# JiangongChen/ORB_SLAM3-1

Measured on AMD Instinct MI355X. Metric: tracking frames/s (ORB extract+match), higher is better.
Workload: dtype u8; 1 GPU; ORBextractor 640x480, 8 levels, 1000 features (configs[1]) + SearchByBoW 1000x1000 per frame (configs[2]); batch_per_gpu=256

## Files before the change

### orb_slam3-1_amd/csrc/orbx_device.h

```cpp
#pragma once

#include <stddef.h>
#include <stdint.h>

#include "../../include/orbslam3_hip.h"

namespace orbx {

constexpr int kEdge = 19;
constexpr int kHalfPatch = 15;
constexpr int kPatch = 31;
constexpr int kMaxLevels = 16;
constexpr int kOctLogFactor = 6;

struct LevelDesc {
    int32_t w, h, stride;
    int32_t nfeat;
    int64_t off;
    int32_t cell_begin, cell_count;
    int32_t cand_off, cand_cap;
    int32_t sel_off, sel_cap;
    float scale;
    int32_t patch_size;
};

struct CellDesc {
    int16_t level;
    int16_t x0, y0, x1, y1;
    int32_t slot_off, slot_cap;
};

struct TileDesc {
    int16_t level, x0, y0, pad;
};

__host__ __device__ inline int xcd_grid(int n_items) { return 8 * ((n_items + 7) / 8); }
__host__ __device__ inline int xcd_remap(int block, int grid, int frame)
{
    const int chunk = grid >> 3;
    return (((block & 7) + frame) & 7) * chunk + (block >> 3);
}

__host__ __device__ inline uint32_t pack_key(uint32_t x, uint32_t y, uint32_t resp) { return (x << 20) | (y << 8) | resp; }
__host__ __device__ inline uint32_t key_x(uint32_t e) { return e >> 20; }
__host__ __device__ inline uint32_t key_y(uint32_t e) { return (e >> 8) & 0xFFFu; }
__host__ __device__ inline uint32_t key_resp(uint32_t e) { return e & 0xFFu; }

}
```

### orb_slam3-1_amd/csrc/orbx_extractor.hip

```cpp
#include <hip/hip_runtime.h>

#include <algorithm>
#include <cmath>
#include <cstdarg>
#include <cstdio>
#include <cstdlib>
#include <cstring>
#include <string>
#include <vector>

#include "hip_check.h"
#include "orbx_kernels.hip"

namespace orbx {

thread_local std::string g_last_error;

int fail(int code, const char* fmt, ...)
{
    char buf[512];
    va_list ap;
    va_start(ap, fmt);
    vsnprintf(buf, sizeof(buf), fmt, ap);
    va_end(ap);
    g_last_error = buf;
    return code;
}

static inline int cv_round_host(double v) { return (int)std::nearbyint(v); }
static inline int cv_floor_host(double v) { int i = (int)v; return i - (i > v); }
static inline int round_up(int v, int a) { return (v + a - 1) / a * a; }

static void gauss_taps_q8(int n, double sigma, int* taps)
{
    std::vector<double> k(n);
    const double scale2x = -0.5 / (sigma * sigma);
    double sum = 0;
    for (int i = 0; i < n; i++) { const double x = i - (n - 1) * 0.5; k[i] = std::exp(scale2x * x * x); sum += k[i]; }
    sum = 1. / sum;
    double err = 0;
    long long acc = 0;
    for (int i = 0; i < n / 2; i++) {
        const double adj = k[i] * sum * 256.0 + err;
        const long long v0 = cv_round_host(adj);
        err = adj - (double)v0;
        taps[i] = taps[n - 1 - i] = (int)v0;
        acc += v0;
    }
    taps[n / 2] = (int)(256 - 2 * acc);
}

template <typename T>
struct DevBuf {
    T* p = nullptr;
    size_t n = 0;
    int ensure(size_t count)
    {
        if (count <= n) return ORBX_OK;
        if (p) { (void)hipFree(p); p = nullptr; n = 0; }
        ORBX_HIP(hipMalloc((void**)&p, count * sizeof(T)));
        n = count;
        return ORBX_OK;
    }
    int upload(const std::vector<T>& v)
    {
        int r = ensure(v.size() ? v.size() : 1);
        if (r) return r;
        if (!v.empty()) ORBX_HIP(hipMemcpy(p, v.data(), v.size() * sizeof(T), hipMemcpyHostToDevice));
        return ORBX_OK;
    }
    void release() { if (p) (void)hipFree(p); p = nullptr; n = 0; }
};

}

using namespace orbx;

struct orbx_extractor {
    int device = 0;
    int nfeatures = 0, nlevels = 0, ini_th = 0, min_th = 0;
    float scale_factor_f = 0;
    double scale_factor_d = 0;
    std::vector<float> scale, inv_scale, sigma2, inv_sigma2;
    std::vector<int> nfeat;
    int taps[7];
    int max_kp = 0;

    int geo_w = 0, geo_h = 0;
    std::vector<LevelDesc> levels;
    std::vector<CellDesc> cells;
    std::vector<TileDesc> tiles;
    size_t pyr_frame_bytes = 0;
    int cand_frame_entries = 0, sel_frame_entries = 0;
    std::vector<StripDesc> strips;
    FastLds fast_layout;
    int fast_corner_cap = 0;
    size_t fast_lds = 0, oct_lds = 0;
    int oct_pool = 0, oct_lds_keys = 0, oct_small_keys = 0;
    bool oct_nodes_hbm = false;
    size_t oct_node_stride = 0;
    size_t oct_small_lds = 0;
    int oct_dyn_keys = 0;
    size_t oct_dyn_lds = 0;
    bool oct_keys_forced = false;

    DevBuf<LevelDesc> d_levels;
    DevBuf<CellDesc> d_cells;
    DevBuf<TileDesc> d_tiles;
    DevBuf<StripDesc> d_strips;
    std::vector<DevBuf<int> > d_qsx0, d_yofs;
    std::vector<DevBuf<uint4> > d_qsel, d_qalpha;
    std::vector<DevBuf<short> > d_ibeta;
    std::vector<DevBuf<int> > d_xofs;
    std::vector<DevBuf<short> > d_ialpha;
    std::vector<uint8_t> resize_generic;

    int batch_cap = 0, last_batch = 0;
    DevBuf<uint8_t> d_pyr, d_blur;
    DevBuf<uint32_t> d_cand, d_scratch, d_sel;
    DevBuf<uint8_t> d_oct_nodes;
    DevBuf<int> d_cell_count, d_sel_count, d_kp_dst;
    DevBuf<OrbxKeyPoint> d_lvl_kps;
    DevBuf<OrbxKeyPoint> d_kps;
    DevBuf<uint8_t> d_desc;
    DevBuf<int> d_n, d_mono, d_status;
    DevBuf<int> d_sad;
    DevBuf<uint8_t> d_stereo_io;
    int out_cap = 0;
    hipStream_t stream = nullptr;
    static constexpr int kProfEvents = 8;
    bool profile = false;
    hipEvent_t prof_ev[kProfEvents] = {};
    int prof_marks = 0;
    hipStream_t prof_stream = nullptr;
    hipStream_t side_stream = nullptr;
    hipEvent_t ev_fork = nullptr, ev_join = nullptr;
    hipStream_t oct_stream = nullptr;
    hipEvent_t ev_oct_join = nullptr, ev_fast0 = nullptr, ev_resize = nullptr;
    hipEvent_t ev_tail = nullptr;
    int dbg_tail_delay_us = 0;
    int last_octree_variant = 0;
    int oct_split = 0, oct_pool_hi = 0;
    size_t oct_lds_hi = 0;
    int split_parts = 1;
    bool serial_schedule = false;
    int resize_tail_first = 4;
    bool oct_dyn_off = false;
    int oct_dyn_max_batch = 64;
    int oct_dyn_keys_beside = 6144;
    bool resize_beside = true;
    std::vector<hipStream_t> aux_streams;
    hipEvent_t ev_parts_fork = nullptr;
    std::vector<hipEvent_t> ev_parts_join;

    int setup_geometry(int w, int h);
    int ensure_batch(int batch);
    int enqueue(const uint8_t* d_imgs, bool level0_ready, int batch, int row_stride, size_t frame_stride,
                int lap0, int lap1, OrbxKeyPoint* o_kps, uint8_t* o_desc, int cap, int* o_n, int* o_mono, int* o_status,
                hipStream_t st);
};

static void build_tables(orbx_extractor* e)
{
    const int nl = e->nlevels;
    e->scale.assign(nl, 1.0f); e->sigma2.assign(nl, 1.0f); e->inv_scale.resize(nl); e->inv_sigma2.resize(nl);
    for (int i = 1; i < nl; i++) {
        e->scale[i] = (float)(e->scale[i - 1] * e->scale_factor_d);
        e->sigma2[i] = e->scale[i] * e->scale[i];
    }
    for (int i = 0; i < nl; i++) {
        e->inv_scale[i] = 1.0f / e->scale[i];
        e->inv_sigma2[i] = 1.0f / e->sigma2[i];
    }
    e->nfeat.resize(nl);
    const float factor = (float)(1.0f / e->scale_factor_d);
    float per_scale = e->nfeatures * (1 - factor) / (1 - (float)std::pow((double)factor, (double)nl));
    int sum = 0;
    for (int l = 0; l < nl - 1; l++) {
        e->nfeat[l] = (int)std::nearbyintf(per_scale);
        sum += e->nfeat[l];
        per_scale *= factor;
    }
    e->nfeat[nl - 1] = std::max(e->nfeatures - sum, 0);
    e->max_kp = 0;
    for (int l = 0; l < nl; l++) e->max_kp += std::max(e->nfeat[l] + 3, 32);
    gauss_taps_q8(7, 2.0, e->taps);
}

int orbx_extractor::setup_geometry(int w, int h)
{
    if (w == geo_w && h == geo_h) return ORBX_OK;
    levels.assign(nlevels, LevelDesc());
    cells.clear();
    tiles.clear();
    strips.clear();
    size_t off = 0;
    int cand_off = 0, sel_off = 0, max_tw = 0, max_th = 0, max_nfeat = 0;
    std::vector<int> node_need(nlevels, 0);
    d_qsx0.resize(nlevels); d_yofs.resize(nlevels); d_qsel.resize(nlevels); d_qalpha.resize(nlevels); d_ibeta.resize(nlevels);
    d_xofs.resize(nlevels); d_ialpha.resize(nlevels); resize_generic.assign(nlevels, 0);
    for (int l = 0; l < nlevels; l++) {
        LevelDesc& L = levels[l];
        L.w = (int)std::nearbyintf((float)w * inv_scale[l]);
        L.h = (int)std::nearbyintf((float)h * inv_scale[l]);
        if (L.w < 1 || L.h < 1) return fail(ORBX_ERR_ARG, "pyramid level %d of a %dx%d image is empty", l, w, h);
        if (L.w > 4096 + 32 || L.h > 4096 + 32) return fail(ORBX_ERR_ARG, "image %dx%d too large (keys are 12-bit)", w, h);
        L.stride = round_up(L.w, 64);
        L.off = (int64_t)off;
        off += (size_t)L.stride * L.h;
        off = (off + 255) & ~(size_t)255;
        L.nfeat = nfeat[l];
        L.scale = scale[l];
        L.patch_size = (int)(kPatch * scale[l]);
        {
            const int bw = (L.w - kEdge + 3) - (kEdge - 3), bh = (L.h - kEdge + 3) - (kEdge - 3);
            const int n_ini = bh > 0 ? (int)std::roundf((float)bw / (float)bh) : 0;
            L.sel_off = sel_off; L.sel_cap = std::max({nfeat[l] + 3, 32, 4 * std::max(n_ini, 0)});
            node_need[l] = std::max(nfeat[l], 4 * std::max(n_ini, 0));
        }
        sel_off += (L.sel_cap + 1) & ~1;
        max_nfeat = std::max(max_nfeat, node_need[l]);
        L.cell_begin = (int)cells.size();
        L.cand_off = cand_off;
        const int minBX = kEdge - 3, minBY = minBX, maxBX = L.w - kEdge + 3, maxBY = L.h - kEdge + 3;
        const float width = (float)(maxBX - minBX), height = (float)(maxBY - minBY);
        const int nCols = (int)(width / 35.f), nRows = (int)(height / 35.f);
        if (nCols > 0 && nRows > 0) {
            const int wCell = (int)std::ceil(width / nCols), hCell = (int)std::ceil(height / nRows);
            for (int i = 0; i < nRows; i++) {
                const float iniY = (float)(minBY + i * hCell);
                float maxY = iniY + hCell + 6;
                if (iniY >= maxBY - 3) continue;
                if (maxY > maxBY) maxY = (float)maxBY;
                for (int j = 0; j < nCols; j++) {
                    const float iniX = (float)(minBX + j * wCell);
                    float maxX = iniX + wCell + 6;
                    if (iniX >= maxBX - 6) continue;
                    if (maxX > maxBX) maxX = (float)maxBX;
                    CellDesc c;
                    c.level = (int16_t)l;
                    c.x0 = (int16_t)iniX; c.x1 = (int16_t)maxX; c.y0 = (int16_t)iniY; c.y1 = (int16_t)maxY;
                    const int iw = c.x1 - c.x0 - 6, ih = c.y1 - c.y0 - 6;
                    if (iw <= 0 || ih <= 0) continue;
                    c.slot_off = cand_off;
                    c.slot_cap = ((iw + 1) / 2) * ((ih + 1) / 2);
                    cand_off += c.slot_cap;
                    max_tw = std::max(max_tw, c.x1 - c.x0);
                    max_th = std::max(max_th, c.y1 - c.y0);
                    cells.push_back(c);
                }
            }
        }
        L.cell_count = (int)cells.size() - L.cell_begin;
        L.cand_cap = cand_off - L.cand_off;
        for (int c0 = L.cell_begin; c0 < (int)cells.size();) {
            int c1 = c0 + 1;
            while (c1 < (int)cells.size() && cells[c1].y0 == cells[c0].y0) c1++;
            const int n_row = c1 - c0;
            const int w_cell = std::max(cells[c0].x1 - cells[c0].x0 - 6, 1);
            static const int strip_width = getenv("ORBX_STRIP_WIDTH") ? std::max(48, std::min(atoi(getenv("ORBX_STRIP_WIDTH")), 250)) : kStripWidth;
            const int per = std::max(1, std::min(kStripMaxCells, (strip_width - 6) / w_cell));
            const int n_strips_row = (n_row + per - 1) / per;
            for (int k = 0; k < n_strips_row; k++) {
                const int a = c0 + (int)((long long)n_row * k / n_strips_row), b = c0 + (int)((long long)n_row * (k + 1) / n_strips_row);
                StripDesc sd;
                sd.level = (int16_t)l; sd.cell0 = (int16_t)a; sd.ncell = (int16_t)(b - a);
                sd.x0 = cells[a].x0; sd.x1 = cells[b - 1].x1; sd.y0 = cells[a].y0; sd.y1 = cells[a].y1; sd.pad = 0;
                strips.push_back(sd);
            }
            c0 = c1;
        }
        for (int y0 = 0; y0 < L.h; y0 += kBlurTH)
            for (int x0 = 0; x0 < L.w; x0 += kBlurTW) {
                TileDesc t; t.level = (int16_t)l; t.x0 = (int16_t)x0; t.y0 = (int16_t)y0; t.pad = 0;
                tiles.push_back(t);
            }
        if (l > 0) {
            const LevelDesc& P = levels[l - 1];
            const double scale_x = 1. / ((double)L.w / P.w), scale_y = 1. / ((double)L.h / P.h);
            const int wpad = round_up(L.w, 4);
            std::vector<int> xofs(wpad, 0), yofs(L.h);
            std::vector<short> ia((size_t)wpad * 2, 0), ib((size_t)L.h * 2);
            auto sat = [](float v) { int iv = (int)std::nearbyintf(v); return (short)std::min(std::max(iv, -32768), 32767); };
            for (int dx = 0; dx < L.w; dx++) {
                float fx = (float)((dx + 0.5) * scale_x - 0.5);
                int sx = cv_floor_host(fx);
                fx -= sx;
                if (sx < 0) { fx = 0; sx = 0; }
                if (sx >= P.w - 1) { fx = 0; sx = P.w - 1; }
                xofs[dx] = sx;
                ia[2 * dx] = sat((1.f - fx) * 2048);
                ia[2 * dx + 1] = sat(fx * 2048);
            }
            for (int dy = 0; dy < L.h; dy++) {
                float fy = (float)((dy + 0.5) * scale_y - 0.5);
                int sy = cv_floor_host(fy);
                fy -= sy;
                yofs[dy] = sy;
                ib[2 * dy] = sat((1.f - fy) * 2048);
                ib[2 * dy + 1] = sat(fy * 2048);
            }
            const int nq = wpad / 4;
            std::vector<int> qsx0(nq);
            std::vector<uint4> qsel(nq), qal(nq);
            for (int q = 0; q < nq; q++) {
                qsx0[q] = xofs[4 * q];
                uint32_t se[4], al[4];
                for (int k = 0; k < 4; k++) {
                    const int dx = 4 * q + k;
                    if (dx < L.w) {
                        const int o = xofs[dx] - qsx0[q];
                        if (o < 0) return fail(ORBX_ERR_INTERNAL, "resize table: source offset %d", o);
                        if (o > 6) { resize_generic[l] = 1; se[k] = 0x0C0C0C0Cu; al[k] = 0u; continue; }
                        se[k] = (uint32_t)o | 0x0C000C00u | ((uint32_t)(o + 1) << 16);
                        al[k] = (uint32_t)(uint16_t)ia[2 * dx] | ((uint32_t)(uint16_t)ia[2 * dx + 1] << 16);
                    } else { se[k] = 0x0C0C0C0Cu; al[k] = 0u; }
                }
                qsel[q] = make_uint4(se[0], se[1], se[2], se[3]);
                qal[q] = make_uint4(al[0], al[1], al[2], al[3]);
            }
            int r;
            if (resize_generic[l] && ((r = d_xofs[l].upload(xofs)) || (r = d_ialpha[l].upload(ia)))) return r;
            if ((r = d_qsx0[l].upload(qsx0)) || (r = d_yofs[l].upload(yofs)) || (r = d_qsel[l].upload(qsel)) || (r = d_qalpha[l].upload(qal)) ||
                (r = d_ibeta[l].upload(ib))) return r;
        }
    }
    pyr_frame_bytes = off;
    cand_frame_entries = std::max(cand_off, 1);
    sel_frame_entries = sel_off;
    {
        if (cells.size() > 32767) return fail(ORBX_ERR_ARG, "%zu FAST cells exceed the strip table's 16-bit cell index", cells.size());
        int max_nch = 1, max_ngx = 1, max_sth = 7, max_ent = 1, max_ncell = 1, max_int = 1;
        for (const StripDesc& sd : strips) {
            const int g0 = (sd.x0 + 3) >> 2, g1 = (sd.x1 - 4) >> 2, ngx = g1 - g0 + 1, sth = sd.y1 - sd.y0, ih = sth - 6;
            if (ngx > 64 || ih > 127) return fail(ORBX_ERR_ARG, "FAST strip of %dx%d px exceeds the 64-quad x 127-row work item index", sd.x1 - sd.x0, sth);
            const int xa = (4 * (g0 - 1)) & ~15, qoff = 4 * g0 - xa;
            max_nch = std::max(max_nch, (qoff + 4 * ngx + 4 + 15) >> 4);
            for (int j = 0; j < sd.ncell; j++) { const CellDesc& c = cells[sd.cell0 + j]; max_int = std::max(max_int, (c.x1 - c.x0 - 6) * ih); }
            max_ngx = std::max(max_ngx, ngx); max_sth = std::max(max_sth, sth);
            max_ent = std::max(max_ent, ((ih + 3) / 4) * (ngx + sd.ncell - 1));
            max_ncell = std::max(max_ncell, (int)sd.ncell);
        }
        if (max_int > 8191) return fail(ORBX_ERR_ARG, "FAST cell interior of %d px exceeds the 8191-px bitmask", max_int);
        FastLds& Z = fast_layout;
        auto al16 = [](size_t v) { return (v + 15) & ~(size_t)15; };
        size_t o = 0;
        Z.tile_pitch = 16 * max_nch;
        o = al16((size_t)max_sth * Z.tile_pitch);
        Z.map_off = (int)o; Z.map_pitch = 4 * max_ngx + 8;
        o = al16(o + (size_t)(max_sth - 6 + 2) * Z.map_pitch);
        Z.colcell_off = (int)o; o = al16(o + Z.map_pitch);
        Z.ent_cap = (max_ent + 7) & ~7;
        Z.ent_off = (int)o; o = al16(o + 2 * 4 * (size_t)Z.ent_cap);
        Z.px_off = (int)o; o = al16(o + 2 * 4 * (size_t)kPxCap);
        Z.corner_cap = fast_corner_cap > 0 ? fast_corner_cap : kCornerCap;
        Z.corner_off = (int)o; o = al16(o + 2 * 4 * (size_t)Z.corner_cap);
        Z.wpc = (max_int + 31) / 32;
        Z.pre_off = (int)o; o = al16(o + 4 * (size_t)max_ncell * Z.wpc);
        Z.bits_off = (int)o; o = al16(o + 4 * (size_t)max_ncell * Z.wpc);
        Z.total = (int)o;
        fast_lds = o;
        if (fast_lds > 150 * 1024) return fail(ORBX_ERR_ARG, "FAST strip of %d quads x %d rows does not fit LDS", max_ngx, max_sth);
    }
    oct_pool = max_nfeat + 16;
    if (oct_pool > 32000) return fail(ORBX_ERR_ARG, "nfeatures per level %d too large for the device octree (16-bit node ids)", max_nfeat);
    const char* env = getenv("ORBX_OCT_LDS_KEYS");
    oct_lds_keys = env ? atoi(env) : 0;
    oct_keys_forced = env != nullptr;
    auto pool_bytes = [](int pool) { return (size_t)pool * (2 * sizeof(SortNode) + 8 + 16 + 2 * kOctLogFactor) + (size_t)((pool + 15) & ~15); };
    const size_t node_bytes = pool_bytes(oct_pool);
    oct_split = 0; oct_pool_hi = 0; oct_lds_hi = 0;
    {
        size_t best = (size_t)nlevels * node_bytes;
        for (int sp = 1; sp < nlevels; sp++) {
            int hi = 0;
            for (int l = sp; l < nlevels; l++) hi = std::max(hi, node_need[l]);
            const size_t cost = (size_t)sp * node_bytes + (size_t)(nlevels - sp) * pool_bytes(hi + 16);
            if (cost < best) { best = cost; oct_split = sp; oct_pool_hi = hi + 16; oct_lds_hi = pool_bytes(hi + 16) + 16; }
        }
    }
    oct_nodes_hbm = node_bytes > 150 * 1024;
    oct_node_stride = (node_bytes + 255) & ~(size_t)255;
    if (oct_nodes_hbm) oct_lds_keys = 0;
    if (!oct_nodes_hbm && node_bytes + 8 * (size_t)oct_lds_keys > 150 * 1024) oct_lds_keys = (int)((150 * 1024 - node_bytes) / 8);
    if (oct_lds_keys < 0) oct_lds_keys = 0;
    oct_lds = node_bytes + 8 * (size_t)oct_lds_keys + 16;
    int max_cand_cap = 0;
    for (const LevelDesc& lv : levels) max_cand_cap = std::max(max_cand_cap, lv.cand_cap);
    oct_small_keys = max_cand_cap;
    if (oct_nodes_hbm || node_bytes + 8 * (size_t)oct_small_keys > 150 * 1024) oct_small_keys = 0;
    oct_small_lds = node_bytes + 8 * (size_t)oct_small_keys + 16;
    if (oct_lds_keys > 0 && oct_lds_keys < max_cand_cap) oct_lds_keys = 0;
    oct_dyn_keys = 0; oct_dyn_lds = 0;
    if (!oct_nodes_hbm && oct_small_keys == 0 && node_bytes + 8 * 2048 <= 150 * 1024) {
        oct_dyn_keys = (int)std::min<size_t>((size_t)max_cand_cap, (150 * 1024 - node_bytes) / 8);
        if (const char* envd = getenv("ORBX_OCT_DYN_KEYS")) oct_dyn_keys = std::max(64, std::min(oct_dyn_keys, atoi(envd)));
        oct_dyn_lds = node_bytes + 8 * (size_t)oct_dyn_keys + 16;
    }
    if (!oct_nodes_hbm) {
        ORBX_HIP(hipFuncSetAttribute((const void*)k_octree<false>, hipFuncAttributeMaxDynamicSharedMemorySize, (int)node_bytes + 64));
        ORBX_HIP(hipFuncSetAttribute((const void*)k_octree<true>, hipFuncAttributeMaxDynamicSharedMemorySize, (int)std::max(oct_lds, oct_small_lds)));
        if (oct_dyn_keys > 0) ORBX_HIP(hipFuncSetAttribute((const void*)k_octree_dyn, hipFuncAttributeMaxDynamicSharedMemorySize, (int)oct_dyn_lds));
    } else {
        oct_lds = 64; oct_small_lds = 64;
    }
    ORBX_HIP(hipFuncSetAttribute((const void*)k_fast_strips, hipFuncAttributeMaxDynamicSharedMemorySize, (int)fast_lds));
    int r;
    if ((r = d_levels.upload(levels)) || (r = d_cells.upload(cells)) || (r = d_tiles.upload(tiles)) || (r = d_strips.upload(strips))) return r;
    geo_w = w; geo_h = h;
    batch_cap = 0;
    return ORBX_OK;
}

int orbx_extractor::ensure_batch(int batch)
{
    if (batch <= batch_cap) return ORBX_OK;
    int r;
    const size_t B = (size_t)batch;
    if ((r = d_pyr.ensure(B * pyr_frame_bytes + 64)) || (r = d_blur.ensure(B * pyr_frame_bytes + 64)) ||
        (r = d_cand.ensure(B * cand_frame_entries)) || (r = d_scratch.ensure(B * 2 * cand_frame_entries)) ||
        (r = d_sel.ensure(B * sel_frame_entries)) || (r = d_cell_count.ensure(B * std::max<size_t>(cells.size(), 1))) ||
        (r = d_sel_count.ensure(B * nlevels)) || (r = d_kp_dst.ensure(B * sel_frame_entries)) ||
        (r = d_lvl_kps.ensure(B * sel_frame_entries)) || (r = d_n.ensure(B)) || (r = d_mono.ensure(B)) || (r = d_status.ensure(B)))
        return r;
    if (oct_nodes_hbm && (r = d_oct_nodes.ensure(B * nlevels * oct_node_stride))) return r;
    ORBX_HIP(hipMemset(d_pyr.p, 0, B * pyr_frame_bytes + 64));
    ORBX_HIP(hipMemset(d_blur.p, 0, B * pyr_frame_bytes + 64));
    batch_cap = batch;
    return ORBX_OK;
}

namespace orbx {
__global__ void k_debug_spin(long long ticks)
{
    const long long t0 = wall_clock64();
    while (wall_clock64() - t0 < ticks) __builtin_amdgcn_s_sleep(32);
}
__global__ __launch_bounds__(256) void k_copy_level0(const uint8_t* __restrict__ src, int row_stride, size_t src_frame_stride,
                                                     uint8_t* __restrict__ pyr, size_t frame_stride, LevelDesc L)
{
    const int x4 = (blockIdx.x * blockDim.x + threadIdx.x) * 4;
    const int y = blockIdx.y;
    if (x4 >= L.w) return;
    const uint8_t* s = src + (size_t)blockIdx.z * src_frame_stride + (size_t)y * row_stride + x4;
    uint32_t v = 0;
#pragma unroll
    for (int k = 0; k < 4; k++) if (x4 + k < L.w) v |= (uint32_t)s[k] << (8 * k);
    *(uint32_t*)(pyr + (size_t)blockIdx.z * frame_stride + L.off + (size_t)y * L.stride + x4) = v;
}
}

int orbx_extractor::enqueue(const uint8_t* d_imgs, bool level0_ready, int batch, int row_stride, size_t frame_stride,
                            int lap0, int lap1, OrbxKeyPoint* o_kps, uint8_t* o_desc, int cap, int* o_n, int* o_mono, int* o_status,
                            hipStream_t st)
{
    const int B = batch;
    ORBX_HIP(hipMemsetAsync(o_status, 0, sizeof(int) * B, st));
    int mark_i = 0;
    auto mark = [&]() { if (profile && mark_i < kProfEvents) (void)hipEventRecord(prof_ev[mark_i++], st); };
#define ORBX_LAUNCHED(name) do { const hipError_t le_ = hipGetLastError(); if (le_ != hipSuccess) return fail(ORBX_ERR_HIP, "launch of %s: %s", name, hipGetErrorString(le_)); } while (0)
    const bool in_place = !level0_ready && ((uintptr_t)d_imgs % 16 == 0) && (row_stride % 16 == 0) && (frame_stride % 16 == 0);
    const int n_cells = (int)cells.size();
    const int quads = (sel_frame_entries + 7) / 8;

    auto run_range = [&](int f0, int nB, hipStream_t s, hipStream_t blur_s, bool marks) -> int {
        uint8_t* pyr = d_pyr.p + (size_t)f0 * pyr_frame_bytes;
        uint8_t* blr = d_blur.p + (size_t)f0 * pyr_frame_bytes;
        SrcImage lvl0;
        lvl0.base = nullptr; lvl0.frame_stride = 0; lvl0.stride = 0; lvl0.w = levels[0].w; lvl0.h = levels[0].h;
        if (in_place) { lvl0.base = d_imgs + (size_t)f0 * frame_stride; lvl0.frame_stride = frame_stride; lvl0.stride = row_stride; }
        if (marks) mark();
        if (!level0_ready && !in_place) {
            const LevelDesc& L0 = levels[0];
            dim3 g((L0.w / 4 + 255) / 256, L0.h, nB);
            hipLaunchKernelGGL(k_copy_level0, g, dim3(256), 0, s, d_imgs + (size_t)f0 * frame_stride, row_stride, frame_stride, pyr, pyr_frame_bytes, L0);
            ORBX_LAUNCHED("k_copy_level0");
        }
        if (marks) mark();
        int l_tail = (nB >= 64 && resize_tail_first >= 2 && resize_tail_first < nlevels) ? resize_tail_first : nlevels;
        for (int l = l_tail; l < nlevels; l++) if (resize_generic[l]) l_tail = nlevels;
        const bool chain_beside = resize_beside && blur_s && oct_stream && n_cells > 0 && l_tail < nlevels && l_tail > 1 &&
                                  !strips.empty() && strips[0].level == 0;
        hipStream_t rs = chain_beside ? oct_stream : s;
        if (chain_beside) { ORBX_HIP(hipEventRecord(ev_fork, s)); ORBX_HIP(hipStreamWaitEvent(rs, ev_fork, 0)); }
        for (int l = 1; l < l_tail; l++) {
            const LevelDesc& D = levels[l];
            dim3 g(xcd_grid(((D.w + kResizeTW - 1) / kResizeTW) * ((D.h + kResizeRows - 1) / kResizeRows)), nB);
            const LevelDesc& P = levels[l - 1];
            SrcImage src;
            src.base = pyr + P.off; src.frame_stride = pyr_frame_bytes; src.stride = P.stride; src.w = P.w; src.h = P.h;
            if (l == 1 && in_place) src = lvl0;
            if (resize_generic[l])
                hipLaunchKernelGGL(k_resize_generic, dim3((D.w + 255) / 256, D.h, nB), dim3(256), 0, rs, src, pyr, pyr_frame_bytes, D,
                                   d_xofs[l].p, d_ialpha[l].p, d_yofs[l].p, d_ibeta[l].p);
            else
            hipLaunchKernelGGL(k_resize, g, dim3(256), 0, rs, src, pyr, pyr_frame_bytes, D,
                               d_qsx0[l].p, d_qsel[l].p, d_qalpha[l].p, d_yofs[l].p, d_ibeta[l].p);
            ORBX_LAUNCHED("k_resize");
        }
        if (chain_beside) ORBX_HIP(hipEventRecord(ev_resize, rs));
        const bool small_batch = !oct_keys_forced && oct_small_keys > 0 && (long long)B * nlevels <= 512;
        const bool dyn_keys = !oct_keys_forced && !small_batch && oct_dyn_keys > 0 && B <= oct_dyn_max_batch && !oct_dyn_off;
        const int dyn_k = (blur_s && B >= 32) ? std::min(oct_dyn_keys, oct_dyn_keys_beside) : oct_dyn_keys;
        const size_t o_lds = small_batch ? oct_small_lds : (dyn_keys ? oct_dyn_lds - 8 * (size_t)(oct_dyn_keys - dyn_k) : oct_lds);
        const int o_keys = small_batch ? oct_small_keys : (dyn_keys ? dyn_k : oct_lds_keys);
        uint32_t* sel = d_sel.p + (size_t)f0 * sel_frame_entries;
        int* sel_cnt = d_sel_count.p + (size_t)f0 * nlevels;
        int* kp_dst = d_kp_dst.p + (size_t)f0 * sel_frame_entries;
        auto oct_kernel = oct_nodes_hbm ? k_octree<false, false> : (dyn_keys ? k_octree_dyn : (o_keys > 0 ? k_octree<true, true> : k_octree<false, true>));
        const bool two_launches = !oct_nodes_hbm && (o_keys == 0 || dyn_keys) && oct_split > 0 && oct_stream && blur_s;
        const int lv_lo = two_launches ? oct_split : nlevels;
        auto launch_octree = [&](hipStream_t qs, int lv0, int lv1, size_t lds, int pool, int keys) {
            if (lv1 > lv0)
                hipLaunchKernelGGL(oct_kernel, dim3(lv1 - lv0, nB), dim3(64), lds, qs, d_levels.p, d_cells.p, d_cand.p + (size_t)f0 * cand_frame_entries, (size_t)cand_frame_entries,
                                   d_cell_count.p + (size_t)f0 * std::max<size_t>(cells.size(), 1), n_cells, d_scratch.p + (size_t)f0 * 2 * cand_frame_entries, (size_t)2 * cand_frame_entries, pool, keys,
                                   sel, sel_frame_entries, sel_cnt, nlevels, o_status + f0,
                                   d_oct_nodes.p ? d_oct_nodes.p + (size_t)f0 * nlevels * oct_node_stride : nullptr, oct_node_stride, lv0);
        };
        auto launch_blur = [&](hipStream_t bs) {
            hipLaunchKernelGGL(k_blur, dim3(xcd_grid((int)tiles.size()), nB), dim3(256), 0, bs, lvl0, pyr, in_place ? pyr : nullptr, blr, pyr_frame_bytes,
                               d_levels.p, d_tiles.p, (int)tiles.size(), taps[0], taps[1], taps[2], taps[3]);
        };
        bool oct0_early = false;
        bool tail_beside = false;
        uint32_t* cand = d_cand.p + (size_t)f0 * cand_frame_entries;
        int* cell_cnt = d_cell_count.p + (size_t)f0 * std::max<size_t>(cells.size(), 1);
        auto launch_fast = [&](hipStream_t fs, int s0, int s1) {
            if (s1 > s0)
                hipLaunchKernelGGL(k_fast_strips, dim3(xcd_grid(s1 - s0), nB), dim3(256), fast_lds, fs, lvl0, pyr, pyr_frame_bytes, d_levels.p, d_cells.p,
                                   d_strips.p + s0, s1 - s0, n_cells, ini_th, min_th, fast_layout, cand, (size_t)cand_frame_entries, cell_cnt);
        };
        int tail_strip = (int)strips.size();
        for (int si = (int)strips.size() - 1; si >= 0 && strips[si].level >= l_tail; si--) tail_strip = si;
        if (l_tail < nlevels) {
            ResizeTables T;
            std::memset(&T, 0, sizeof(T));
            for (int l = l_tail; l < nlevels; l++) { T.q_sx0[l] = d_qsx0[l].p; T.q_sel[l] = d_qsel[l].p; T.q_alpha[l] = d_qalpha[l].p; T.yofs[l] = d_yofs[l].p; T.ibeta[l] = d_ibeta[l].p; }
            const bool beside = blur_s && oct_stream && n_cells > 0 && tail_strip > 0;
            hipStream_t ts = beside ? oct_stream : s;
            if (beside && !chain_beside) { ORBX_HIP(hipEventRecord(ev_fork, s)); ORBX_HIP(hipStreamWaitEvent(ts, ev_fork, 0)); }
            if (dbg_tail_delay_us > 0) hipLaunchKernelGGL(k_debug_spin, dim3(1), dim3(64), 0, ts, (long long)dbg_tail_delay_us * 100);
            hipLaunchKernelGGL(k_resize_tail, dim3(nB), dim3(1024), 0, ts, pyr, pyr_frame_bytes, d_levels.p, T, l_tail, nlevels);
            ORBX_LAUNCHED("k_resize_tail");
            if (beside) {
                ORBX_HIP(hipEventRecord(ev_tail, ts));
                tail_beside = true;
                launch_fast(ts, tail_strip, (int)strips.size());
                ORBX_HIP(hipEventRecord(ev_oct_join, ts));
                int l1_strip = tail_strip;
                for (int si = tail_strip - 1; si >= 0 && strips[si].level >= 1; si--) l1_strip = si;
                if (two_launches && oct_split > 1 && l1_strip > 0 && l1_strip < tail_strip) {
                    launch_fast(s, 0, l1_strip);
                    ORBX_HIP(hipEventRecord(ev_fast0, s));
                    ORBX_HIP(hipStreamWaitEvent(blur_s, ev_fast0, 0));
                    launch_octree(blur_s, 0, 1, o_lds, oct_pool, o_keys);
                    oct0_early = true;
                    if (chain_beside) ORBX_HIP(hipStreamWaitEvent(s, ev_resize, 0));
                    launch_fast(s, l1_strip, tail_strip);
                } else if (chain_beside && l1_strip > 0 && l1_strip < tail_strip) {
                    launch_fast(s, 0, l1_strip);
                    ORBX_HIP(hipStreamWaitEvent(s, ev_resize, 0));
                    launch_fast(s, l1_strip, tail_strip);
                } else {
                    if (chain_beside) ORBX_HIP(hipStreamWaitEvent(s, ev_resize, 0));
                    launch_fast(s, 0, tail_strip);
                }
                ORBX_HIP(hipStreamWaitEvent(blur_s, ev_oct_join, 0));
            } else {
                if (marks) mark();
                if (n_cells > 0) launch_fast(s, 0, (int)strips.size());
            }
        } else {
            if (marks) mark();
            if (n_cells > 0) launch_fast(s, 0, (int)strips.size());
        }
        ORBX_LAUNCHED("k_fast_strips");
        if (marks) mark();
        hipStream_t os = blur_s ? blur_s : s;
        if (blur_s) {
            ORBX_HIP(hipEventRecord(ev_fork, s));
            ORBX_HIP(hipStreamWaitEvent(blur_s, ev_fork, 0));
        }
        if (two_launches) {
            ORBX_HIP(hipStreamWaitEvent(oct_stream, ev_fork, 0));
            {
                const int k_hi = dyn_keys ? std::max(64, o_keys / 2) : 0;
                launch_octree(oct_stream, oct_split, nlevels, oct_lds_hi + 8 * (size_t)k_hi, oct_pool_hi, k_hi);
            }
            ORBX_HIP(hipEventRecord(ev_oct_join, oct_stream));
        }
        launch_octree(os, oct0_early ? 1 : 0, lv_lo, o_lds, oct_pool, o_keys);
        if (blur_s) {
            if (tail_beside) ORBX_HIP(hipStreamWaitEvent(s, ev_tail, 0));
            launch_blur(s);
        }
        last_octree_variant = (oct_nodes_hbm ? 0 : (dyn_keys ? 3 : (o_keys > 0 ? 1 : 2))) | (two_launches ? 4 : 0) | (oct0_early ? 8 : 0) | (in_place ? 16 : 0) | (tail_beside ? 32 : 0) | (chain_beside ? 64 : 0);
        if (two_launches) ORBX_HIP(hipStreamWaitEvent(os, ev_oct_join, 0));
        ORBX_LAUNCHED("k_octree / k_blur");
        if (marks) mark();
        hipLaunchKernelGGL(k_index, dim3(nB), dim3(64), 0, os, d_levels.p, nlevels, sel, sel_frame_entries, sel_cnt,
                           lap0, lap1, cap, kp_dst, sel_frame_entries, o_n + f0, o_mono + f0, o_status + f0);
        ORBX_LAUNCHED("k_index");
        if (marks) mark();
        if (blur_s) { ORBX_HIP(hipEventRecord(ev_join, blur_s)); ORBX_HIP(hipStreamWaitEvent(s, ev_join, 0)); }
        else launch_blur(s);
        if (marks) mark();
        hipLaunchKernelGGL(k_orient_desc, dim3((unsigned)(((long long)quads * nB + 7) / 8 * 8)), dim3(256), 0, s, pyr, blr, pyr_frame_bytes,
                           d_levels.p, nlevels, sel, sel_frame_entries, sel_cnt, kp_dst, sel_frame_entries,
                           o_kps + (size_t)f0 * cap, o_desc + (size_t)f0 * cap * 32, cap, d_lvl_kps.p + (size_t)f0 * sel_frame_entries, quads, nB);
        ORBX_LAUNCHED("k_orient_desc");
        if (marks) mark();
        return ORBX_OK;
    };

    int parts = 1;
    if (!profile && split_parts > 1 && B >= 32 * split_parts) parts = std::min(split_parts, 1 + (int)aux_streams.size());
    int r;
    if (parts == 1) {
        if ((r = run_range(0, B, st, (!profile && !serial_schedule && side_stream && B >= 32) ? side_stream : nullptr, true))) return r;
    } else {
        ORBX_HIP(hipEventRecord(ev_parts_fork, st));
        for (int p = 0; p < parts; p++) {
            const int f0 = (int)((long long)B * p / parts), f1 = (int)((long long)B * (p + 1) / parts);
            hipStream_t s = p == 0 ? st : aux_streams[p - 1];
            if (p > 0) ORBX_HIP(hipStreamWaitEvent(s, ev_parts_fork, 0));
            if ((r = run_range(f0, f1 - f0, s, nullptr, false))) return r;
            if (p > 0) { ORBX_HIP(hipEventRecord(ev_parts_join[p - 1], s)); ORBX_HIP(hipStreamWaitEvent(st, ev_parts_join[p - 1], 0)); }
        }
    }
    prof_marks = mark_i;
    prof_stream = st;
    ORBX_HIP(hipGetLastError());
    last_batch = B;
    return ORBX_OK;
}

extern "C" {

int orbx_profile_enable(orbx_extractor* e, int on)
{
    if (!e) return fail(ORBX_ERR_ARG, "NULL handle");
    ORBX_HIP(hipSetDevice(e->device));
    if (on && !e->prof_ev[0])
        for (int i = 0; i < orbx_extractor::kProfEvents; i++) ORBX_HIP(hipEventCreate(&e->prof_ev[i]));
    e->profile = on != 0;
    e->prof_marks = 0;
    return ORBX_OK;
}

int orbx_profile_read(orbx_extractor* e, float* stage_ms, int n_stages)
{
    if (!e || !stage_ms) return fail(ORBX_ERR_ARG, "NULL argument");
    if (!e->profile || e->prof_marks < 2) return fail(ORBX_ERR_ARG, "profiling was not enabled for the last call");
    ORBX_HIP(hipSetDevice(e->device));
    ORBX_HIP(hipStreamSynchronize(e->prof_stream));
    for (int i = 0; i < n_stages; i++) {
        stage_ms[i] = 0.f;
        if (i + 1 < e->prof_marks) ORBX_HIP(hipEventElapsedTime(&stage_ms[i], e->prof_ev[i], e->prof_ev[i + 1]));
    }
    return ORBX_OK;
}

const char* orbx_last_error(void) { return g_last_error.c_str(); }

int orbx_device_count(void)
{
    int n = 0;
    if (hipGetDeviceCount(&n) != hipSuccess) return 0;
    return n;
}

int orbx_create(int nfeatures, float scale_factor, int nlevels, int ini_th_fast, int min_th_fast, int device, orbx_extractor** out)
{
    if (!out) return fail(ORBX_ERR_ARG, "out is NULL");
    *out = nullptr;
    if (nlevels < 1 || nlevels > kMaxLevels || nfeatures < 1 || !(scale_factor > 1.0f))
        return fail(ORBX_ERR_ARG, "bad extractor parameters (nfeatures=%d scale=%f nlevels=%d)", nfeatures, scale_factor, nlevels);
    if (int r = stage::check_device(device)) return r;
    ORBX_HIP(hipSetDevice(device));
    orbx_extractor* e = new orbx_extractor();
    e->device = device;
    e->nfeatures = nfeatures; e->nlevels = nlevels; e->ini_th = ini_th_fast; e->min_th = min_th_fast;
    e->scale_factor_f = scale_factor; e->scale_factor_d = (double)scale_factor;
    build_tables(e);
    if (hipStreamCreateWithFlags(&e->stream, hipStreamNonBlocking) != hipSuccess) { delete e; return fail(ORBX_ERR_HIP, "stream create failed"); }
    if (hipStreamCreateWithFlags(&e->side_stream, hipStreamNonBlocking) != hipSuccess ||
        hipEventCreateWithFlags(&e->ev_fork, hipEventDisableTiming) != hipSuccess ||
        hipEventCreateWithFlags(&e->ev_join, hipEventDisableTiming) != hipSuccess ||
        hipEventCreateWithFlags(&e->ev_parts_fork, hipEventDisableTiming) != hipSuccess ||
        hipStreamCreateWithFlags(&e->oct_stream, hipStreamNonBlocking) != hipSuccess ||
        hipEventCreateWithFlags(&e->ev_oct_join, hipEventDisableTiming) != hipSuccess ||
        hipEventCreateWithFlags(&e->ev_tail, hipEventDisableTiming) != hipSuccess ||
        hipEventCreateWithFlags(&e->ev_resize, hipEventDisableTiming) != hipSuccess ||
        hipEventCreateWithFlags(&e->ev_fast0, hipEventDisableTiming) != hipSuccess) { orbx_destroy(e); return fail(ORBX_ERR_HIP, "side stream create failed"); }
    if (const char* env = getenv("ORBX_SERIAL")) e->serial_schedule = atoi(env) != 0;
    if (const char* env = getenv("ORBX_SPLIT")) e->split_parts = std::max(1, std::min(atoi(env), 4));
    if (const char* env = getenv("ORBX_RESIZE_TAIL")) e->resize_tail_first = atoi(env);
    if (const char* env = getenv("ORBX_RESIZE_BESIDE")) e->resize_beside = atoi(env) != 0;
    if (const char* env = getenv("ORBX_OCT_DYN")) e->oct_dyn_off = atoi(env) == 0;
    if (const char* env = getenv("ORBX_OCT_DYN_MAXB")) e->oct_dyn_max_batch = atoi(env);
    if (const char* env = getenv("ORBX_OCT_DYN_KEYS_BESIDE")) e->oct_dyn_keys_beside = std::max(64, atoi(env));
    for (int i = 0; i + 1 < e->split_parts; i++) {
        hipStream_t s = nullptr; hipEvent_t ev = nullptr;
        if (hipStreamCreateWithFlags(&s, hipStreamNonBlocking) != hipSuccess || hipEventCreateWithFlags(&ev, hipEventDisableTiming) != hipSuccess) {
            if (s) (void)hipStreamDestroy(s);
            break;
        }
        e->aux_streams.push_back(s); e->ev_parts_join.push_back(ev);
    }
    *out = e;
    return ORBX_OK;
}

void orbx_destroy(orbx_extractor* e)
{
    if (!e) return;
    (void)hipSetDevice(e->device);
    if (e->stream) { (void)hipStreamSynchronize(e->stream); (void)hipStreamDestroy(e->stream); }
    if (e->side_stream) { (void)hipStreamSynchronize(e->side_stream); (void)hipStreamDestroy(e->side_stream); }
    if (e->oct_stream) { (void)hipStreamSynchronize(e->oct_stream); (void)hipStreamDestroy(e->oct_stream); }
    if (e->ev_oct_join) (void)hipEventDestroy(e->ev_oct_join);
    if (e->ev_fast0) (void)hipEventDestroy(e->ev_fast0);
    if (e->ev_resize) (void)hipEventDestroy(e->ev_resize);
    if (e->ev_tail) (void)hipEventDestroy(e->ev_tail);
    if (e->ev_fork) (void)hipEventDestroy(e->ev_fork);
    if (e->ev_join) (void)hipEventDestroy(e->ev_join);
    for (hipStream_t s : e->aux_streams) { (void)hipStreamSynchronize(s); (void)hipStreamDestroy(s); }
    for (hipEvent_t ev : e->ev_parts_join) (void)hipEventDestroy(ev);
    if (e->ev_parts_fork) (void)hipEventDestroy(e->ev_parts_fork);
    e->d_levels.release(); e->d_cells.release(); e->d_tiles.release(); e->d_strips.release();
    for (auto& b : e->d_qsx0) b.release();
    for (auto& b : e->d_yofs) b.release();
    for (auto& b : e->d_qsel) b.release();
    for (auto& b : e->d_qalpha) b.release();
    for (auto& b : e->d_ibeta) b.release();
    for (auto& b : e->d_xofs) b.release();
    for (auto& b : e->d_ialpha) b.release();
    e->d_pyr.release(); e->d_blur.release(); e->d_cand.release(); e->d_scratch.release(); e->d_sel.release(); e->d_oct_nodes.release();
    e->d_cell_count.release(); e->d_sel_count.release(); e->d_kp_dst.release(); e->d_lvl_kps.release();
    e->d_kps.release(); e->d_desc.release(); e->d_n.release(); e->d_mono.release(); e->d_status.release();
    e->d_sad.release(); e->d_stereo_io.release();
    delete e;
}

int orbx_max_keypoints(const orbx_extractor* e) { return e ? e->max_kp : 0; }

int orbx_max_keypoints_for(const orbx_extractor* e, int width, int height)
{
    if (!e || width < 1 || height < 1) return 0;
    int total = 0;
    for (int l = 0; l < e->nlevels; l++) {
        const int lw = (int)std::nearbyintf((float)width * e->inv_scale[l]), lh = (int)std::nearbyintf((float)height * e->inv_scale[l]);
        const int bw = (lw - kEdge + 3) - (kEdge - 3), bh = (lh - kEdge + 3) - (kEdge - 3);
        const int n_ini = bh > 0 ? (int)std::roundf((float)bw / (float)bh) : 0;
        total += std::max({e->nfeat[l] + 3, 32, 4 * std::max(n_ini, 0)});
    }
    return total;
}
int orbx_levels(const orbx_extractor* e) { return e ? e->nlevels : 0; }
float orbx_scale_factor(const orbx_extractor* e) { return e ? e->scale_factor_f : 0.f; }

int orbx_scale_tables(const orbx_extractor* e, float* scale, float* inv_scale, float* sigma2, float* inv_sigma2)
{
    if (!e) return fail(ORBX_ERR_ARG, "NULL handle");
    for (int i = 0; i < e->nlevels; i++) {
        if (scale) scale[i] = e->scale[i];
        if (inv_scale) inv_scale[i] = e->inv_scale[i];
        if (sigma2) sigma2[i] = e->sigma2[i];
        if (inv_sigma2) inv_sigma2[i] = e->inv_sigma2[i];
    }
    return ORBX_OK;
}

int orbx_features_per_level(const orbx_extractor* e, int* n_per_level)
{
    if (!e || !n_per_level) return fail(ORBX_ERR_ARG, "NULL argument");
    for (int i = 0; i < e->nlevels; i++) n_per_level[i] = e->nfeat[i];
    return ORBX_OK;
}

int orbx_extract_batch_device(orbx_extractor* e, const uint8_t* d_imgs, int batch, int width, int height,
                              int row_stride, size_t frame_stride, int lap0, int lap1,
                              OrbxKeyPoint* d_kps, uint8_t* d_desc, int cap, int32_t* d_n, int32_t* d_mono,
                              int32_t* d_status, void* stream)
{
    if (!e || !d_imgs || !d_kps || !d_desc || !d_n || !d_mono || !d_status) return fail(ORBX_ERR_ARG, "NULL argument");
    if (batch < 1 || width < 1 || height < 1 || row_stride < width || cap < 1) return fail(ORBX_ERR_ARG, "bad batch/geometry");
    ORBX_HIP(hipSetDevice(e->device));
    int r;
    if ((r = e->setup_geometry(width, height)) || (r = e->ensure_batch(batch))) return r;
    return e->enqueue(d_imgs, false, batch, row_stride, frame_stride, lap0, lap1, d_kps, d_desc, cap, d_n, d_mono, d_status,
                      (hipStream_t)stream);
}

int orbx_extract_batch(orbx_extractor* e, const uint8_t* const* imgs, int batch, int width, int height, int stride,
                       int lap0, int lap1, OrbxKeyPoint* kps, uint8_t* desc, int cap, int* n, int* mono_index)
{
    if (!e || !imgs || !kps || !desc || !n || !mono_index) return fail(ORBX_ERR_ARG, "NULL argument");
    if (batch < 1 || cap < 1) return fail(ORBX_ERR_ARG, "bad batch/capacity");
    if (width < 1 || height < 1) { for (int b = 0; b < batch; b++) { n[b] = 0; mono_index[b] = -1; } return ORBX_ERR_EMPTY; }
    if (stride < width) return fail(ORBX_ERR_ARG, "stride < width");
    ORBX_HIP(hipSetDevice(e->device));
    int r;
    if ((r = e->setup_geometry(width, height)) || (r = e->ensure_batch(batch))) return r;
    const size_t B = (size_t)batch;
    if ((r = e->d_kps.ensure(B * cap)) || (r = e->d_desc.ensure(B * cap * 32))) return r;
    const LevelDesc& L0 = e->levels[0];
    for (int b = 0; b < batch; b++) {
        if (!imgs[b]) return fail(ORBX_ERR_ARG, "imgs[%d] is NULL", b);
        ORBX_HIP(hipMemcpy2DAsync(e->d_pyr.p + b * e->pyr_frame_bytes + L0.off, L0.stride, imgs[b], stride, width, height,
                                  hipMemcpyHostToDevice, e->stream));
    }
    if ((r = e->enqueue(nullptr, true, batch, 0, 0, lap0, lap1, e->d_kps.p, e->d_desc.p, cap, e->d_n.p, e->d_mono.p, e->d_status.p, e->stream)))
        return r;
    std::vector<int> st(batch);
    ORBX_HIP(hipMemcpyAsync(n, e->d_n.p, sizeof(int) * B, hipMemcpyDeviceToHost, e->stream));
    ORBX_HIP(hipMemcpyAsync(mono_index, e->d_mono.p, sizeof(int) * B, hipMemcpyDeviceToHost, e->stream));
    ORBX_HIP(hipMemcpyAsync(st.data(), e->d_status.p, sizeof(int) * B, hipMemcpyDeviceToHost, e->stream));
    ORBX_HIP(hipMemcpyAsync(kps, e->d_kps.p, sizeof(OrbxKeyPoint) * B * cap, hipMemcpyDeviceToHost, e->stream));
    ORBX_HIP(hipMemcpyAsync(desc, e->d_desc.p, B * cap * 32, hipMemcpyDeviceToHost, e->stream));
    ORBX_HIP(hipStreamSynchronize(e->stream));
    for (int b = 0; b < batch; b++)
        if (st[b] != ORBX_OK) return fail(st[b], "frame %d: device status %d (n=%d, cap=%d)", b, st[b], n[b], cap);
    return ORBX_OK;
}

int orbx_extract(orbx_extractor* e, const uint8_t* img, int width, int height, int stride,
                 int lap0, int lap1, OrbxKeyPoint* kps, uint8_t* desc, int cap, int* n, int* mono_index)
{
    if (!img || width < 1 || height < 1) {
        if (n) *n = 0;
        if (mono_index) *mono_index = -1;
        return ORBX_ERR_EMPTY;
    }
    const uint8_t* imgs[1] = {img};
    return orbx_extract_batch(e, imgs, 1, width, height, stride, lap0, lap1, kps, desc, cap, n, mono_index);
}

int orbx_pyramid_level_size(const orbx_extractor* e, int level, int* width, int* height)
{
    if (!e || level < 0 || level >= e->nlevels || e->geo_w == 0) return fail(ORBX_ERR_ARG, "no pyramid (level %d)", level);
    if (width) *width = e->levels[level].w;
    if (height) *height = e->levels[level].h;
    return ORBX_OK;
}

static int download_level(orbx_extractor* e, const uint8_t* base, int frame, int level, int border, uint8_t* dst, int dst_stride)
{
    if (!e || !dst || level < 0 || level >= e->nlevels || frame < 0 || frame >= e->last_batch || border < 0)
        return fail(ORBX_ERR_ARG, "bad frame/level");
    const LevelDesc& L = e->levels[level];
    if (dst_stride < L.w + 2 * border) return fail(ORBX_ERR_ARG, "dst_stride too small");
    ORBX_HIP(hipSetDevice(e->device));
    ORBX_HIP(hipStreamSynchronize(e->stream));
    ORBX_HIP(hipMemcpy2D(dst + (size_t)border * dst_stride + border, dst_stride, base + (size_t)frame * e->pyr_frame_bytes + L.off,
                         L.stride, L.w, L.h, hipMemcpyDeviceToHost));
    if (border > 0) {
        auto refl = [](int p, int len) { if (len == 1) return 0; while (p < 0 || p >= len) p = p < 0 ? -p : 2 * len - 2 - p; return p; };
        for (int y = 0; y < L.h + 2 * border; y++) {
            const int sy = refl(y - border, L.h) + border;
            uint8_t* row = dst + (size_t)y * dst_stride;
            const uint8_t* srow = dst + (size_t)sy * dst_stride;
            if (sy != y) std::memcpy(row + border, srow + border, L.w);
            for (int x = 0; x < border; x++) {
                row[x] = row[border + refl(x - border, L.w)];
                row[border + L.w + x] = row[border + refl(L.w + x, L.w)];
            }
        }
    }
    return ORBX_OK;
}

int orbx_pyramid_level(orbx_extractor* e, int frame, int level, int border, uint8_t* dst, int dst_stride)
{
    return download_level(e, e ? e->d_pyr.p : nullptr, frame, level, border, dst, dst_stride);
}

int orbx_debug_blurred_level(orbx_extractor* e, int frame, int level, uint8_t* dst, int dst_stride)
{
    return download_level(e, e ? e->d_blur.p : nullptr, frame, level, 0, dst, dst_stride);
}

int orbx_debug_candidates(orbx_extractor* e, int frame, int level, OrbxKeyPoint* out, int cap, int* n)
{
    if (!e || !out || !n || level < 0 || level >= e->nlevels || frame < 0 || frame >= e->last_batch) return fail(ORBX_ERR_ARG, "bad frame/level");
    ORBX_HIP(hipSetDevice(e->device));
    ORBX_HIP(hipStreamSynchronize(e->stream));
    const LevelDesc& L = e->levels[level];
    std::vector<int> cnt(std::max(L.cell_count, 1));
    std::vector<uint32_t> ent(std::max(L.cand_cap, 1));
    if (L.cell_count > 0) {
        ORBX_HIP(hipMemcpy(cnt.data(), e->d_cell_count.p + (size_t)frame * e->cells.size() + L.cell_begin, sizeof(int) * L.cell_count, hipMemcpyDeviceToHost));
        ORBX_HIP(hipMemcpy(ent.data(), e->d_cand.p + (size_t)frame * e->cand_frame_entries + L.cand_off, sizeof(uint32_t) * L.cand_cap, hipMemcpyDeviceToHost));
    }
    int k = 0;
    for (int c = 0; c < L.cell_count; c++) {
        const CellDesc& cd = e->cells[L.cell_begin + c];
        for (int i = 0; i < cnt[c]; i++, k++) {
            if (k >= cap) continue;
            const uint32_t en = ent[cd.slot_off - L.cand_off + i];
            OrbxKeyPoint kp;
            kp.x = (float)key_x(en); kp.y = (float)key_y(en); kp.size = 7.f; kp.angle = -1.f; kp.response = (float)key_resp(en);
            kp.octave = 0; kp.class_id = -1;
            out[k] = kp;
        }
    }
    *n = k;
    return ORBX_OK;
}

int orbx_debug_level_keypoints(orbx_extractor* e, int frame, int level, OrbxKeyPoint* out, int cap, int* n)
{
    if (!e || !out || !n || level < 0 || level >= e->nlevels || frame < 0 || frame >= e->last_batch) return fail(ORBX_ERR_ARG, "bad frame/level");
    ORBX_HIP(hipSetDevice(e->device));
    ORBX_HIP(hipStreamSynchronize(e->stream));
    const LevelDesc& L = e->levels[level];
    int cnt = 0;
    ORBX_HIP(hipMemcpy(&cnt, e->d_sel_count.p + (size_t)frame * e->nlevels + level, sizeof(int), hipMemcpyDeviceToHost));
    *n = cnt;
    const int m = std::min(cnt, cap);
    if (m > 0)
        ORBX_HIP(hipMemcpy(out, e->d_lvl_kps.p + (size_t)frame * e->sel_frame_entries + L.sel_off, sizeof(OrbxKeyPoint) * m, hipMemcpyDeviceToHost));
    return ORBX_OK;
}

int orbx_debug_set_tail_delay(orbx_extractor* e, int microseconds)
{
    if (!e || microseconds < 0 || microseconds > 20000) return fail(ORBX_ERR_ARG, "bad tail delay");
    e->dbg_tail_delay_us = microseconds;
    return ORBX_OK;
}

int orbx_debug_last_schedule(orbx_extractor* e)
{
    if (!e) return fail(ORBX_ERR_ARG, "NULL handle");
    return e->last_octree_variant;
}

int orbx_debug_set_fast_corner_cap(orbx_extractor* e, int cap)
{
    if (!e) return fail(ORBX_ERR_ARG, "NULL handle");
    e->fast_corner_cap = cap > 0 ? std::min(cap, 4096) : 0;
    e->geo_w = e->geo_h = 0;
    return ORBX_OK;
}

int orbx_debug_introsort(int32_t* count, int32_t* ulx, int32_t* node, int n)
{
    if (n < 0) return ORBX_ERR_ARG;
    std::vector<SortNode> v(n);
    for (int i = 0; i < n; i++) { v[i].count = count[i]; v[i].ulx = ulx[i]; v[i].node = node[i]; }
    std::vector<int> stack(3 * kIntrosortStack);
    introsort_nodes(v.data(), n, stack.data());
    for (int i = 0; i < n; i++) { count[i] = v[i].count; ulx[i] = v[i].ulx; node[i] = v[i].node; }
    return ORBX_OK;
}

int orbx_debug_wave_sort(int32_t* count, int32_t* ulx, int32_t* node, int n)
{
    if (n < 0 || n > 4000) return fail(ORBX_ERR_ARG, "n %d outside 0..4000", n);
    if (n == 0) return ORBX_OK;
    std::vector<SortNode> v(n);
    for (int i = 0; i < n; i++) { v[i].count = count[i]; v[i].ulx = ulx[i]; v[i].node = node[i]; }
    SortNode* d = nullptr;
    ORBX_HIP(hipMalloc(&d, sizeof(SortNode) * n));
    int r = ORBX_OK;
    const size_t lds = 2 * sizeof(SortNode) * (size_t)n + 2 * (size_t)n + 16;
    if (hipMemcpy(d, v.data(), sizeof(SortNode) * n, hipMemcpyHostToDevice) != hipSuccess) r = ORBX_ERR_HIP;
    if (!r && hipFuncSetAttribute((const void*)k_debug_wave_sort, hipFuncAttributeMaxDynamicSharedMemorySize, (int)lds) != hipSuccess) r = ORBX_ERR_HIP;
    if (!r) {
        hipLaunchKernelGGL(k_debug_wave_sort, dim3(1), dim3(64), lds, 0, d, n);
        if (hipGetLastError() != hipSuccess || hipDeviceSynchronize() != hipSuccess) r = ORBX_ERR_HIP;
    }
    if (!r && hipMemcpy(v.data(), d, sizeof(SortNode) * n, hipMemcpyDeviceToHost) != hipSuccess) r = ORBX_ERR_HIP;
    (void)hipFree(d);
    if (r) return fail(r, "device sort failed");
    for (int i = 0; i < n; i++) { count[i] = v[i].count; ulx[i] = v[i].ulx; node[i] = v[i].node; }
    return ORBX_OK;
}

static int stereo_enqueue(orbx_extractor* l, orbx_extractor* r, int frame0, int batch,
                          const OrbxKeyPoint* d_kps_l, const uint8_t* d_desc_l, const int32_t* d_n_l,
                          const OrbxKeyPoint* d_kps_r, const uint8_t* d_desc_r, const int32_t* d_n_r, int cap,
                          float mb, float mbf, float* d_u_right, float* d_depth, hipStream_t st)
{
    if (l->geo_w == 0 || l->geo_w != r->geo_w || l->geo_h != r->geo_h || l->nlevels != r->nlevels || l->scale_factor_f != r->scale_factor_f)
        return fail(ORBX_ERR_ARG, "the two extractors do not hold pyramids of the same geometry");
    if (l->device != r->device) return fail(ORBX_ERR_ARG, "the two extractors live on different devices");
    if (frame0 < 0 || batch < 1 || frame0 + batch > l->last_batch || frame0 + batch > r->last_batch) return fail(ORBX_ERR_ARG, "frames outside the last extract call");
    if (l->nlevels > 16) return fail(ORBX_ERR_ARG, "more than 16 pyramid levels");
    if (cap < 1 || cap > 8192) return fail(ORBX_ERR_ARG, "cap %d outside 1..8192", cap);
    if (!(mb > 0.f) || !(mbf > 0.f)) return fail(ORBX_ERR_ARG, "mb and mbf must be positive");
    int rr = l->d_sad.ensure((size_t)batch * cap);
    if (rr) return rr;
    StereoTables T;
    for (int i = 0; i < 16; i++) { T.scale[i] = l->scale[std::min(i, l->nlevels - 1)]; T.inv_scale[i] = l->inv_scale[std::min(i, l->nlevels - 1)]; }
    const uint8_t* pl = l->d_pyr.p + (size_t)frame0 * l->pyr_frame_bytes;
    const uint8_t* pr = r->d_pyr.p + (size_t)frame0 * r->pyr_frame_bytes;
    hipLaunchKernelGGL(k_stereo_match, dim3((cap + 3) / 4, batch), dim3(256), 0, st, pl, pr, l->pyr_frame_bytes, l->d_levels.p, T,
                       d_kps_l, d_desc_l, d_n_l, d_kps_r, d_desc_r, d_n_r, cap, mb, mbf, l->nlevels, d_u_right, d_depth, l->d_sad.p);
    int n_pow2 = 2;
    while (n_pow2 < cap) n_pow2 <<= 1;
    hipLaunchKernelGGL(k_stereo_median, dim3(batch), dim3(256), (size_t)n_pow2 * sizeof(int), st, d_n_l, cap, n_pow2, d_u_right, d_depth, l->d_sad.p);
    ORBX_HIP(hipGetLastError());
    return ORBX_OK;
}

int orbx_stereo_matches_device(orbx_extractor* left, orbx_extractor* right, int batch,
                               const OrbxKeyPoint* d_kps_l, const uint8_t* d_desc_l, const int32_t* d_n_l,
                               const OrbxKeyPoint* d_kps_r, const uint8_t* d_desc_r, const int32_t* d_n_r, int cap,
                               float mb, float mbf, float* d_u_right, float* d_depth, void* stream)
{
    if (!left || !right || !d_kps_l || !d_desc_l || !d_n_l || !d_kps_r || !d_desc_r || !d_n_r || !d_u_right || !d_depth) return fail(ORBX_ERR_ARG, "NULL argument");
    ORBX_HIP(hipSetDevice(left->device));
    return stereo_enqueue(left, right, 0, batch, d_kps_l, d_desc_l, d_n_l, d_kps_r, d_desc_r, d_n_r, cap, mb, mbf, d_u_right, d_depth, (hipStream_t)stream);
}

int orbx_stereo_matches(orbx_extractor* left, orbx_extractor* right, int frame,
                        const OrbxKeyPoint* kps_l, const uint8_t* desc_l, int n_l,
                        const OrbxKeyPoint* kps_r, const uint8_t* desc_r, int n_r, float mb, float mbf, float* u_right, float* depth)
{
    if (!left || !right || n_l < 0 || n_r < 0 || (n_l > 0 && (!kps_l || !desc_l || !u_right || !depth)) || (n_r > 0 && (!kps_r || !desc_r)))
        return fail(ORBX_ERR_ARG, "NULL argument");
    if (n_l == 0) return ORBX_OK;
    ORBX_HIP(hipSetDevice(left->device));
    const int cap = std::max(std::max(n_l, n_r), 1);
    auto al = [](size_t v) { return (v + 255) & ~(size_t)255; };
    const size_t o_kl = 0, o_dl = al(o_kl + sizeof(OrbxKeyPoint) * (size_t)cap), o_kr = al(o_dl + 32 * (size_t)cap), o_dr = al(o_kr + sizeof(OrbxKeyPoint) * (size_t)cap),
                 o_n = al(o_dr + 32 * (size_t)cap), o_u = al(o_n + 8), o_d = al(o_u + 4 * (size_t)cap), total = al(o_d + 4 * (size_t)cap);
    int r = left->d_stereo_io.ensure(total);
    if (r) return r;
    uint8_t* b = left->d_stereo_io.p;
    hipStream_t st = left->stream;
    const int32_t nn[2] = {n_l, n_r};
    ORBX_HIP(hipMemcpyAsync(b + o_kl, kps_l, sizeof(OrbxKeyPoint) * (size_t)n_l, hipMemcpyHostToDevice, st));
    ORBX_HIP(hipMemcpyAsync(b + o_dl, desc_l, 32 * (size_t)n_l, hipMemcpyHostToDevice, st));
    if (n_r > 0) {
        ORBX_HIP(hipMemcpyAsync(b + o_kr, kps_r, sizeof(OrbxKeyPoint) * (size_t)n_r, hipMemcpyHostToDevice, st));
        ORBX_HIP(hipMemcpyAsync(b + o_dr, desc_r, 32 * (size_t)n_r, hipMemcpyHostToDevice, st));
    }
    ORBX_HIP(hipMemcpyAsync(b + o_n, nn, 8, hipMemcpyHostToDevice, st));
    ORBX_HIP(hipStreamSynchronize(right->stream));
    r = stereo_enqueue(left, right, frame, 1, (const OrbxKeyPoint*)(b + o_kl), b + o_dl, (const int32_t*)(b + o_n),
                       (const OrbxKeyPoint*)(b + o_kr), b + o_dr, (const int32_t*)(b + o_n) + 1, cap, mb, mbf, (float*)(b + o_u), (float*)(b + o_d), st);
    if (r) return r;
    ORBX_HIP(hipMemcpyAsync(u_right, b + o_u, 4 * (size_t)n_l, hipMemcpyDeviceToHost, st));
    ORBX_HIP(hipMemcpyAsync(depth, b + o_d, 4 * (size_t)n_l, hipMemcpyDeviceToHost, st));
    ORBX_HIP(hipStreamSynchronize(st));
    return ORBX_OK;
}

float orbx_debug_fast_atan2(float y, float x) { return fast_atan2_deg(y, x); }
void orbx_debug_sincos(float a, float* c, float* s) { sincos_f32(a, c, s); }

#ifdef ORBX_FAST_TIMING
int orbx_debug_fast_prof(unsigned long long* out16)
{
    unsigned long long z[16] = {0};
    if (hipMemcpyFromSymbol(out16, HIP_SYMBOL(d_fast_prof), sizeof(z)) != hipSuccess) return ORBX_ERR_HIP;
    if (hipMemcpyToSymbol(HIP_SYMBOL(d_fast_prof), z, sizeof(z)) != hipSuccess) return ORBX_ERR_HIP;
    return ORBX_OK;
}
#endif
#ifdef ORBX_OCT_TIMING
int orbx_debug_oct_prof(unsigned long long* out10)
{
    if (hipMemcpyFromSymbol(out10, HIP_SYMBOL(d_oct_prof), 10 * sizeof(unsigned long long)) != hipSuccess) return ORBX_ERR_HIP;
    return ORBX_OK;
}
#endif


}
```

### orb_slam3-1_amd/csrc/orbx_kernels.hip

```cpp
#include <hip/hip_runtime.h>
#include <stdint.h>

#include "orbx_device.h"
#include "orbx_introsort.h"
#include "orbx_math.h"

namespace orbx {

__device__ __align__(16) const signed char d_pattern[1024] = {
#include "orb_pattern_31.inc"
};

typedef unsigned short us2 __attribute__((ext_vector_type(2)));
__device__ __forceinline__ us2 as_us2(uint32_t v) { return __builtin_bit_cast(us2, v); }
__device__ __forceinline__ uint32_t as_u32(us2 v) { return __builtin_bit_cast(uint32_t, v); }

struct SrcImage {
    const uint8_t* base;
    size_t frame_stride;
    int32_t stride, w, h;
};

struct __attribute__((aligned(4))) Dwords3 { uint32_t x, y, z; };
struct __attribute__((aligned(4))) Dwords4 { uint32_t x, y, z, w; };
constexpr int kResizeRows = 64, kResizeTW = 64;

__device__ __forceinline__ void resize_tile(const SrcImage& src, uint8_t* __restrict__ pyr, size_t frame_stride, const LevelDesc& dst,
                                            const int* __restrict__ q_sx0, const uint4* __restrict__ q_sel, const uint4* __restrict__ q_alpha,
                                            const int* __restrict__ yofs, const short* __restrict__ ibeta, int tile, int frame, int lane, int wave)
{
    const int tiles_x = (dst.w + kResizeTW - 1) / kResizeTW;
    const int ty = tile / tiles_x, tx = tile - ty * tiles_x;
    const int q = tx * (kResizeTW / 4) + (lane & 15), rsel = lane >> 4;
    if (4 * q >= dst.w) return;
    const int sx0 = q_sx0[q];
    const uint4 sel = q_sel[q], al = q_alpha[q];
    const uint32_t sels[4] = {sel.x, sel.y, sel.z, sel.w}, als[4] = {al.x, al.y, al.z, al.w};
    const int a = sx0 & ~3;
    const uint32_t sh = (uint32_t)(sx0 & 3);
    const int last = src.stride - 4;
    const int o0 = a, o1 = min(a + 4, last), o2 = min(a + 8, last);
    const uint8_t* S = src.base + (size_t)frame * src.frame_stride;
    uint8_t* D = pyr + (size_t)frame * frame_stride + dst.off + 4 * q;
    constexpr int NR = kResizeRows / 16;
    const int dy0 = ty * kResizeRows + wave * (kResizeRows / 4) + rsel;
    uint32_t u[NR][3], v[NR][3], bb[NR];
#pragma unroll
    for (int r = 0; r < NR; r++) {
        const int dy = min(dy0 + 4 * r, dst.h - 1);
        const int sy = yofs[dy];
        const int sy0 = min(max(sy, 0), src.h - 1), sy1 = min(max(sy + 1, 0), src.h - 1);
        bb[r] = ((const uint32_t*)ibeta)[dy];
        const uint8_t* r0p = S + (size_t)sy0 * src.stride;
        const uint8_t* r1p = S + (size_t)sy1 * src.stride;
        if (a + 8 <= last) {
            const Dwords3 tu = *(const Dwords3*)(r0p + a), tv = *(const Dwords3*)(r1p + a);
            u[r][0] = tu.x; u[r][1] = tu.y; u[r][2] = tu.z;
            v[r][0] = tv.x; v[r][1] = tv.y; v[r][2] = tv.z;
        } else {
            u[r][0] = *(const uint32_t*)(r0p + o0); u[r][1] = *(const uint32_t*)(r0p + o1); u[r][2] = *(const uint32_t*)(r0p + o2);
            v[r][0] = *(const uint32_t*)(r1p + o0); v[r][1] = *(const uint32_t*)(r1p + o1); v[r][2] = *(const uint32_t*)(r1p + o2);
        }
    }
#pragma unroll
    for (int r = 0; r < NR; r++) {
        const int dy = dy0 + 4 * r;
        if (dy >= dst.h) continue;
        const uint32_t b0 = bb[r] & 0xFFFFu, b1 = bb[r] >> 16;
        const uint32_t ulo = __builtin_amdgcn_alignbyte(u[r][1], u[r][0], sh), uhi = __builtin_amdgcn_alignbyte(u[r][2], u[r][1], sh);
        const uint32_t vlo = __builtin_amdgcn_alignbyte(v[r][1], v[r][0], sh), vhi = __builtin_amdgcn_alignbyte(v[r][2], v[r][1], sh);
        uint32_t out[4];
#pragma unroll
        for (int k = 0; k < 4; k++) {
            const us2 ak = as_us2(als[k]);
            const uint32_t h0 = __builtin_amdgcn_udot2(as_us2(__builtin_amdgcn_perm(uhi, ulo, sels[k])), ak, 0u, false);
            const uint32_t h1 = __builtin_amdgcn_udot2(as_us2(__builtin_amdgcn_perm(vhi, vlo, sels[k])), ak, 0u, false);
            const uint32_t val = ((__umul24(b0, h0 >> 4) >> 16) + (__umul24(b1, h1 >> 4) >> 16) + 2u) >> 2;
            out[k] = min(val, 255u);
        }
        *(uint32_t*)(D + (size_t)dy * dst.stride) = out[0] | (out[1] << 8) | (out[2] << 16) | (out[3] << 24);
    }
}

__global__ __launch_bounds__(256) void k_resize(SrcImage src, uint8_t* __restrict__ pyr, size_t frame_stride, LevelDesc dst,
                                                const int* __restrict__ q_sx0, const uint4* __restrict__ q_sel, const uint4* __restrict__ q_alpha,
                                                const int* __restrict__ yofs, const short* __restrict__ ibeta)
{
    const int tiles_x = (dst.w + kResizeTW - 1) / kResizeTW, tiles_y = (dst.h + kResizeRows - 1) / kResizeRows;
    const int tile = xcd_remap(blockIdx.x, gridDim.x, blockIdx.y);
    if (tile >= tiles_x * tiles_y) return;
    resize_tile(src, pyr, frame_stride, dst, q_sx0, q_sel, q_alpha, yofs, ibeta, tile, blockIdx.y, threadIdx.x & 63,
                __builtin_amdgcn_readfirstlane(threadIdx.x >> 6));
}

__global__ __launch_bounds__(256) void k_resize_generic(SrcImage src, uint8_t* __restrict__ pyr, size_t frame_stride, LevelDesc dst,
                                                        const int* __restrict__ xofs, const short* __restrict__ ialpha,
                                                        const int* __restrict__ yofs, const short* __restrict__ ibeta)
{
    const int dx = blockIdx.x * blockDim.x + threadIdx.x, dy = blockIdx.y, frame = blockIdx.z;
    if (dx >= dst.w) return;
    const uint8_t* S = src.base + (size_t)frame * src.frame_stride;
    const int sx = xofs[dx], sy = yofs[dy];
    const uint32_t a0 = (uint16_t)ialpha[2 * dx], a1 = (uint16_t)ialpha[2 * dx + 1];
    const uint32_t b0 = (uint16_t)ibeta[2 * dy], b1 = (uint16_t)ibeta[2 * dy + 1];
    const int sy0 = min(max(sy, 0), src.h - 1), sy1 = min(max(sy + 1, 0), src.h - 1);
    const int sx1 = min(sx + 1, src.w - 1);
    const uint8_t* r0 = S + (size_t)sy0 * src.stride;
    const uint8_t* r1 = S + (size_t)sy1 * src.stride;
    const uint32_t h0 = r0[sx] * a0 + r0[sx1] * a1, h1 = r1[sx] * a0 + r1[sx1] * a1;
    const uint32_t val = ((__umul24(b0, h0 >> 4) >> 16) + (__umul24(b1, h1 >> 4) >> 16) + 2u) >> 2;
    pyr[(size_t)frame * frame_stride + dst.off + (size_t)dy * dst.stride + dx] = (uint8_t)min(val, 255u);
}

struct ResizeTables {
    const int* q_sx0[kMaxLevels]; const uint4* q_sel[kMaxLevels]; const uint4* q_alpha[kMaxLevels];
    const int* yofs[kMaxLevels]; const short* ibeta[kMaxLevels];
};
__global__ __launch_bounds__(1024) void k_resize_tail(uint8_t* __restrict__ pyr, size_t frame_stride, const LevelDesc* __restrict__ levels,
                                                      ResizeTables T, int l_first, int n_levels)
{
    const int frame = blockIdx.x;
    const int sub = __builtin_amdgcn_readfirstlane(threadIdx.x >> 8), wave = __builtin_amdgcn_readfirstlane((threadIdx.x >> 6) & 3);
    const int lane = threadIdx.x & 63;
    for (int l = l_first; l < n_levels; l++) {
        const LevelDesc D = levels[l], P = levels[l - 1];
        SrcImage src;
        src.base = pyr + P.off; src.frame_stride = frame_stride; src.stride = P.stride; src.w = P.w; src.h = P.h;
        const int tiles = ((D.w + kResizeTW - 1) / kResizeTW) * ((D.h + kResizeRows - 1) / kResizeRows);
        for (int t = sub; t < tiles; t += 4)
            resize_tile(src, pyr, frame_stride, D, T.q_sx0[l], T.q_sel[l], T.q_alpha[l], T.yofs[l], T.ibeta[l], t, frame, lane, wave);
        __syncthreads();
    }
}

#include "orbx_fast_strips.inc"

#ifdef ORBX_OCT_TIMING
__device__ unsigned long long d_oct_prof[10];
#endif
struct OctLds {
    short* ulx; short* uly; short* brx; short* bry;
    int* beg; int* cnt;
    int* pidx; short* freelist; short* order;
    short* plog;
    uint8_t* flg;
};

template <bool LDS_KEYS, bool LDS_NODES>
__device__ __forceinline__ void octree_body(const LevelDesc* __restrict__ levels, const CellDesc* __restrict__ cells,
                                            const uint32_t* __restrict__ cand, size_t cand_frame_stride,
                                            const int* __restrict__ cell_count, int n_cells,
                                            uint32_t* __restrict__ scratch, size_t scratch_frame_stride,
                                            int pool, int lds_keys_cap,
                                            uint32_t* __restrict__ sel, int sel_frame_stride,
                                            int* __restrict__ sel_count, int n_levels, int* __restrict__ status,
                                            uint8_t* __restrict__ node_scratch, size_t node_stride, int level_first,
                                            uint8_t* __restrict__ smem, int* __restrict__ s_sort_stack)
{
    static_assert(LDS_NODES || !LDS_KEYS, "a pool too large for LDS leaves no room for LDS keys");
    const int level = level_first + blockIdx.x, frame = blockIdx.y;
    const int lane = threadIdx.x;
    const LevelDesc L = levels[level];
    const int N = L.nfeat;
    const unsigned long long lt = (1ull << lane) - 1ull;
#ifdef ORBX_OCT_TIMING
    long long tq[8] = {0, 0, 0, 0, 0, 0, 0, 0};
    const bool timed = level == 0 && frame == 0 && lane == 0;
    long long t_prev = clock64();
    const long long t_kernel0 = t_prev;
    int n_div = 0;
#define ORBX_OTICK(k) if (timed) { const long long t_now = clock64(); tq[k] += t_now - t_prev; t_prev = t_now; }
#else
#define ORBX_OTICK(k)
#endif

    OctLds S;
    uint8_t* p;
    if constexpr (LDS_NODES) p = smem;
    else p = node_scratch + ((size_t)blockIdx.y * gridDim.x + blockIdx.x) * node_stride;
    SortNode* const ex_new = (SortNode*)p; p += sizeof(SortNode) * pool;
    SortNode* const ex_sorted = (SortNode*)p; p += sizeof(SortNode) * pool;
    S.beg = (int*)p; p += 4 * pool;
    S.cnt = (int*)p; p += 4 * pool;
    S.ulx = (short*)p; p += 2 * pool;  S.uly = (short*)p; p += 2 * pool;
    S.brx = (short*)p; p += 2 * pool;  S.bry = (short*)p; p += 2 * pool;
    S.pidx = (int*)p; p += 4 * pool;
    S.freelist = (short*)p; p += 2 * pool; S.order = (short*)p; p += 2 * pool;
    S.plog = (short*)p; p += 2 * kOctLogFactor * pool;
    S.flg = p; p += (pool + 15) & ~15;
    uint32_t* kb;
    int cap;
    if constexpr (LDS_KEYS) { kb = (uint32_t*)p; cap = lds_keys_cap; }
    else { kb = scratch + (size_t)frame * scratch_frame_stride + 2 * (size_t)L.cand_off; cap = L.cand_cap; }

    int* out_count = sel_count + (size_t)frame * n_levels + level;
    uint32_t* out = sel + (size_t)frame * sel_frame_stride + L.sel_off;

    const uint32_t* fc = cand + (size_t)frame * cand_frame_stride;
    const int* cc = cell_count + (size_t)frame * n_cells;
    int total = 0;
    for (int c0 = 0; c0 < L.cell_count; c0 += 64) {
        const int ci = c0 + lane;
        int n = 0, slot_off = 0;
        if (ci < L.cell_count) { n = cc[L.cell_begin + ci]; slot_off = cells[L.cell_begin + ci].slot_off; }
        const int incl = wave_incl_scan(n);
        const int base = total + incl - n;
        if (base + n > cap) n = 0;
        for (int k = 0; __ballot(k < n) != 0ull; k += 8) {
            uint32_t e[8];
#pragma unroll
            for (int u = 0; u < 8; u++) e[u] = (k + u < n) ? fc[slot_off + k + u] : 0u;
#pragma unroll
            for (int u = 0; u < 8; u++) if (k + u < n) kb[base + k + u] = e[u];
        }
        total += __builtin_amdgcn_readlane(incl, 63);
    }
    if (total > cap) {
        if (lane == 0) { atomicExch(status + frame, ORBX_ERR_INTERNAL); *out_count = 0; }
        return;
    }
    __syncthreads();
    ORBX_OTICK(0)

    const int width = (L.w - kEdge + 3) - (kEdge - 3), height = (L.h - kEdge + 3) - (kEdge - 3);
    const int nIni = (height > 0) ? (int)roundf((float)width / (float)height) : 0;
    if (total == 0 || nIni <= 0 || nIni > pool / 2) {
        if (lane == 0) {
            *out_count = 0;
            if (total != 0 && nIni > pool / 2) atomicExch(status + frame, ORBX_ERR_INTERNAL);
        }
        return;
    }

    const int plog_cap = kOctLogFactor * pool;
    int np = 0, size = 0, nfree = pool, n_ex = 0;
    for (int i = lane; i < pool; i += 64) S.freelist[i] = (short)(pool - 1 - i);
    __syncthreads();
    bool overflow = false;
    auto compact = [&]() {
        int w = 0;
        for (int i0 = 0; i0 < np; i0 += 64) {
            const int i = i0 + lane;
            const int id = (i < np) ? (int)S.plog[i] : -1;
            const unsigned long long m = __ballot(id >= 0);
            if (id >= 0) { const int pos = w + __popcll(m & lt); S.plog[pos] = (short)id; S.pidx[id] = pos; }
            w += __popcll(m);
        }
        np = w;
        __syncthreads();
    };

    const float hX = (float)width / (float)nIni;
    if (nIni == 1) {
        if (lane == 0) {
            const int id = S.freelist[nfree - 1];
            S.ulx[id] = 0; S.uly[id] = 0; S.brx[id] = (short)(int)hX; S.bry[id] = (short)height;
            S.beg[id] = 0; S.cnt[id] = total; S.flg[id] = (uint8_t)(total == 1 ? 1 : 0);
            S.plog[0] = (short)id; S.pidx[id] = 0;
        }
        nfree--; np = 1; size = 1;
        __syncthreads();
    } else {
        int strip_beg = 0;
        for (int s = 0; s < nIni; s++) {
            int cnt = 0;
            for (int k0 = 0; k0 < total; k0 += 64) {
                const int k = k0 + lane;
                bool in = false;
                uint32_t e = 0;
                if (k < total) { e = kb[k]; in = ((int)((float)key_x(e) / hX) == s); }
                const unsigned long long m = __ballot(in);
                if (in) kb[cap + strip_beg + cnt + __popcll(m & lt)] = e;
                cnt += __popcll(m);
            }
            int id = -1;
            if (cnt > 0) {
                id = S.freelist[--nfree];
                if (lane == 0) {
                    S.ulx[id] = (short)(int)(hX * (float)s);       S.uly[id] = 0;
                    S.brx[id] = (short)(int)(hX * (float)(s + 1)); S.bry[id] = (short)height;
                    S.beg[id] = strip_beg; S.cnt[id] = cnt;
                    S.flg[id] = (uint8_t)(2 | (cnt == 1 ? 1 : 0));
                }
            }
            if (lane == 0) S.order[s] = (short)id;
            strip_beg += cnt;
        }
        __syncthreads();
        for (int s = nIni - 1; s >= 0; s--) {
            const int id = S.order[s];
            if (id >= 0) { if (lane == 0) { S.plog[np] = (short)id; S.pidx[id] = np; } np++; size++; }
        }
        __syncthreads();
    }
    ORBX_OTICK(1)

    auto divide_batch = [&](const int id, const bool sorted_phase, int& n_to_expand) -> bool {
        const bool act = id >= 0;
        int ulx = 0, uly = 0, brx = 0, bry = 0, beg = 0, cnt = 0, src = 0;
        if (act) {
            ulx = S.ulx[id]; uly = S.uly[id]; brx = S.brx[id]; bry = S.bry[id];
            beg = S.beg[id]; cnt = S.cnt[id]; src = (S.flg[id] >> 1) & 1;
        }
        const int halfX = (brx - ulx + 1) >> 1;
        const int halfY = (bry - uly + 1) >> 1;
        const int midx = ulx + halfX, midy = uly + halfY;
        const int in_off = (src ? cap : 0) + beg, out_off = (src ? 0 : cap) + beg;
        const unsigned long long m_act = __ballot(act);
        const int small_max = (__popcll(m_act) <= 6) ? 0 : 32;
        const bool small = act && cnt <= small_max;
        int c0 = 0, c1 = 0, c2 = 0, c3 = 0;
        if (__ballot(small) != 0ull) {
            for (int k = 0; __ballot(small && k < cnt) != 0ull; k += 4) {
#pragma unroll
                for (int u = 0; u < 4; u++) {
                    if (small && k + u < cnt) {
                        const uint32_t e = kb[in_off + k + u];
                        const int cls = ((int)key_x(e) >= midx ? 1 : 0) + ((int)key_y(e) >= midy ? 2 : 0);
                        c0 += cls == 0; c1 += cls == 1; c2 += cls == 2; c3 += cls == 3;
                    }
                }
            }
            int w0 = out_off, w1 = out_off + c0, w2 = w1 + c1, w3 = w2 + c2;
            for (int k = 0; __ballot(small && k < cnt) != 0ull; k += 4) {
                uint32_t e[4];
#pragma unroll
                for (int u = 0; u < 4; u++) e[u] = (small && k + u < cnt) ? kb[in_off + k + u] : 0u;
#pragma unroll
                for (int u = 0; u < 4; u++) {
                    if (small && k + u < cnt) {
                        const bool r = (int)key_x(e[u]) >= midx, d = (int)key_y(e[u]) >= midy;
                        const int pos = d ? (r ? w3 : w2) : (r ? w1 : w0);
                        kb[pos] = e[u];
                        w0 += (!d && !r); w1 += (!d && r); w2 += (d && !r); w3 += (d && r);
                    }
                }
            }
        }
        for (unsigned long long mb = __ballot(act && !small); mb != 0ull; mb &= mb - 1ull) {
            const int b = __builtin_ctzll(mb);
            const int bin = __builtin_amdgcn_readlane(in_off, b), bout = __builtin_amdgcn_readlane(out_off, b);
            const int bcnt = __builtin_amdgcn_readlane(cnt, b);
            const int bmx = __builtin_amdgcn_readlane(midx, b), bmy = __builtin_amdgcn_readlane(midy, b);
            int s0 = 0, s1 = 0, s2 = 0, s3 = 0;
            if (bcnt <= 64) {
                int cls = -1;
                uint32_t e = 0;
                if (lane < bcnt) { e = kb[bin + lane]; cls = ((int)key_x(e) >= bmx ? 1 : 0) + ((int)key_y(e) >= bmy ? 2 : 0); }
                const unsigned long long m0 = __ballot(cls == 0), m1 = __ballot(cls == 1), m2 = __ballot(cls == 2), m3 = __ballot(cls == 3);
                s0 = __popcll(m0); s1 = __popcll(m1); s2 = __popcll(m2); s3 = __popcll(m3);
                const unsigned long long mm = (cls == 0) ? m0 : (cls == 1) ? m1 : (cls == 2) ? m2 : m3;
                const int basec = (cls == 0) ? 0 : (cls == 1) ? s0 : (cls == 2) ? s0 + s1 : s0 + s1 + s2;
                if (cls >= 0) kb[bout + basec + __popcll(mm & lt)] = e;
            } else {
                for (int k0 = 0; k0 < bcnt; k0 += 256) {
                    uint32_t e[4];
#pragma unroll
                    for (int u = 0; u < 4; u++) { const int k = k0 + 64 * u + lane; e[u] = (k < bcnt) ? kb[bin + k] : 0u; }
#pragma unroll
                    for (int u = 0; u < 4; u++) {
                        const int k = k0 + 64 * u + lane;
                        const int cls = (k < bcnt) ? ((int)key_x(e[u]) >= bmx ? 1 : 0) + ((int)key_y(e[u]) >= bmy ? 2 : 0) : -1;
                        s0 += __popcll(__ballot(cls == 0)); s1 += __popcll(__ballot(cls == 1));
                        s2 += __popcll(__ballot(cls == 2)); s3 += __popcll(__ballot(cls == 3));
                    }
                }
                int w0 = bout, w1 = bout + s0, w2 = w1 + s1, w3 = w2 + s2;
                for (int k0 = 0; k0 < bcnt; k0 += 256) {
                    uint32_t e[4];
#pragma unroll
                    for (int u = 0; u < 4; u++) { const int k = k0 + 64 * u + lane; e[u] = (k < bcnt) ? kb[bin + k] : 0u; }
#pragma unroll
                    for (int u = 0; u < 4; u++) {
                        const int k = k0 + 64 * u + lane;
                        const int cls = (k < bcnt) ? ((int)key_x(e[u]) >= bmx ? 1 : 0) + ((int)key_y(e[u]) >= bmy ? 2 : 0) : -1;
                        const unsigned long long m0 = __ballot(cls == 0), m1 = __ballot(cls == 1), m2 = __ballot(cls == 2), m3 = __ballot(cls == 3);
                        const unsigned long long mm = (cls == 0) ? m0 : (cls == 1) ? m1 : (cls == 2) ? m2 : m3;
                        const int wc = (cls == 0) ? w0 : (cls == 1) ? w1 : (cls == 2) ? w2 : w3;
                        if (cls >= 0) kb[wc + __popcll(mm & lt)] = e[u];
                        w0 += __popcll(m0); w1 += __popcll(m1); w2 += __popcll(m2); w3 += __popcll(m3);
                    }
                }
            }
            if (lane == b) { c0 = s0; c1 = s1; c2 = s2; c3 = s3; }
        }
        ORBX_OTICK(2)

        bool keep = act, reached = false;
        if (sorted_phase) {
            const int grow = act ? (c0 > 0) + (c1 > 0) + (c2 > 0) + (c3 > 0) - 1 : 0;
            const int incl_g = wave_incl_scan(grow);
            const unsigned long long hit = __ballot(act && size + incl_g >= N);
            if (hit != 0ull) { reached = true; keep = act && lane <= __builtin_ctzll(hit); }
        }
        for (unsigned long long rem = __ballot(keep); rem != 0ull;) {
            const bool in = (rem >> lane) & 1ull;
            const int ne = in ? (c0 > 0) + (c1 > 0) + (c2 > 0) + (c3 > 0) : 0;
            const int nx = in ? (c0 > 1) + (c1 > 1) + (c2 > 1) + (c3 > 1) : 0;
            const int incl_e = wave_incl_scan(ne), incl_x = wave_incl_scan(nx), incl_a = wave_incl_scan(in ? 1 : 0);
            const bool take = in && incl_e <= nfree;
            const unsigned long long m_take = __ballot(take);
            if (m_take == 0ull) { overflow = true; return true; }
            const int last = 63 - __builtin_clzll(m_take);
            const int tot_e = __builtin_amdgcn_readlane(incl_e, last), tot_x = __builtin_amdgcn_readlane(incl_x, last), tot_a = __builtin_amdgcn_readlane(incl_a, last);
            if (np + tot_e > plog_cap || n_ex + tot_x > pool) { overflow = true; return true; }
            if (take) {
                int slot = np + incl_e - ne, fl = nfree - 1 - (incl_e - ne), xs = n_ex + incl_x - nx, cb = beg;
#pragma unroll
                for (int c = 0; c < 4; c++) {
                    const int cn = (c == 0) ? c0 : (c == 1) ? c1 : (c == 2) ? c2 : c3;
                    if (cn > 0) {
                        const int ch = S.freelist[fl--];
                        const int ux = (c & 1) ? midx : ulx, uy = (c & 2) ? midy : uly;
                        S.ulx[ch] = (short)ux; S.uly[ch] = (short)uy;
                        S.brx[ch] = (short)((c & 1) ? brx : midx); S.bry[ch] = (short)((c & 2) ? bry : midy);
                        S.beg[ch] = cb; S.cnt[ch] = cn;
                        S.flg[ch] = (uint8_t)(((src ^ 1) << 1) | (cn == 1 ? 1 : 0));
                        S.plog[slot] = (short)ch; S.pidx[ch] = slot; slot++;
                        if (cn > 1) { SortNode sn; sn.count = cn; sn.ulx = ux; sn.node = ch; ex_new[xs++] = sn; }
                        cb += cn;
                    }
                }
                S.plog[S.pidx[id]] = -1;
            }
            __syncthreads();
            np += tot_e; size += tot_e - tot_a; nfree -= tot_e;
            if (take) S.freelist[nfree + incl_a - 1] = (short)id;
            nfree += tot_a;
            n_to_expand += tot_x; n_ex += tot_x;
#ifdef ORBX_OCT_TIMING
            n_div += tot_a;
#endif
            rem &= ~m_take;
            __syncthreads();
        }
        ORBX_OTICK(3)
        return reached;
    };

    bool finish = false;
    int guard = 0;
    while (!finish && !overflow && guard++ < 64) {
        const int prev_size = size;
        int n_to_expand = 0;
        n_ex = 0;
        compact();
        const int np0 = np;
        for (int b0 = 0; b0 < np0 && !overflow; b0 += 64) {
            const int idx = np0 - 1 - (b0 + lane);
            int id = -1;
            if (idx >= 0) { const int cur = S.plog[idx]; if (cur >= 0 && !(S.flg[cur] & 1)) id = cur; }
            if (__ballot(id >= 0) != 0ull) divide_batch(id, false, n_to_expand);
        }
        if (size >= N || size == prev_size) {
            finish = true;
        } else if (size + n_to_expand * 3 > N) {
            int guard2 = 0;
            while (!finish && !overflow && guard2++ < 4096) {
                const int prev_size2 = size;
                compact();
                const int n_prev = min(n_ex, pool);
                ORBX_OTICK(4)
                wave_sort_nodes(ex_new, ex_sorted, n_prev, s_sort_stack, S.order);
                ORBX_OTICK(5)
                n_ex = 0;
                int dummy = 0;
                for (int b0 = 0; b0 < n_prev && !overflow; b0 += 64) {
                    const int j = n_prev - 1 - (b0 + lane);
                    const int id = (j >= 0) ? ex_sorted[j].node : -1;
                    if (divide_batch(id, true, dummy)) break;
                }
                if (size >= N || size == prev_size2) finish = true;
            }
        }
    }
    if (overflow) {
        if (lane == 0) { atomicExch(status + frame, ORBX_ERR_INTERNAL); *out_count = 0; }
        return;
    }
    ORBX_OTICK(4)

    compact();
    for (int k = lane; k < np && k < pool; k += 64) S.order[k] = S.plog[np - 1 - k];
    __syncthreads();
    const int n_out = min(size, L.sel_cap);
    for (int k0 = 0; k0 < n_out; k0 += 64) {
        const int k = k0 + lane;
        int off = 0, cnt = 0;
        if (k < n_out) { const int id = S.order[k]; off = (((S.flg[id] >> 1) & 1) ? cap : 0) + S.beg[id]; cnt = S.cnt[id]; }
        uint32_t best = 0;
        for (int i = 0; __ballot(i < cnt) != 0ull; i += 4) {
            uint32_t e[4];
#pragma unroll
            for (int u = 0; u < 4; u++) e[u] = (i + u < cnt) ? kb[off + i + u] : 0u;
#pragma unroll
            for (int u = 0; u < 4; u++) if (i + u < cnt && (i + u == 0 || key_resp(e[u]) > key_resp(best))) best = e[u];
        }
        if (k < n_out) out[k] = best;
    }
    if (lane == 0) {
        *out_count = n_out;
        if (size > L.sel_cap) atomicExch(status + frame, ORBX_ERR_INTERNAL);
    }
    ORBX_OTICK(6)
#ifdef ORBX_OCT_TIMING
    if (timed) {
        for (int i = 0; i < 7; i++) d_oct_prof[i] = (unsigned long long)tq[i];
        d_oct_prof[7] = (unsigned long long)(clock64() - t_kernel0);
        d_oct_prof[8] = (unsigned long long)total; d_oct_prof[9] = (unsigned long long)n_div;
    }
#endif
}

template <bool LDS_KEYS, bool LDS_NODES = true>
__global__ __launch_bounds__(64) void k_octree(const LevelDesc* __restrict__ levels, const CellDesc* __restrict__ cells,
                                               const uint32_t* __restrict__ cand, size_t cand_frame_stride,
                                               const int* __restrict__ cell_count, int n_cells,
                                               uint32_t* __restrict__ scratch, size_t scratch_frame_stride,
                                               int pool, int lds_keys_cap,
                                               uint32_t* __restrict__ sel, int sel_frame_stride,
                                               int* __restrict__ sel_count, int n_levels, int* __restrict__ status,
                                               uint8_t* __restrict__ node_scratch, size_t node_stride, int level_first)
{
    extern __shared__ __align__(16) uint8_t smem[];
    __shared__ int s_sort_stack[3 * kIntrosortStack];
    octree_body<LDS_KEYS, LDS_NODES>(levels, cells, cand, cand_frame_stride, cell_count, n_cells, scratch, scratch_frame_stride, pool, lds_keys_cap,
                                     sel, sel_frame_stride, sel_count, n_levels, status, node_scratch, node_stride, level_first, smem, s_sort_stack);
}

__global__ __launch_bounds__(64) void k_octree_dyn(const LevelDesc* __restrict__ levels, const CellDesc* __restrict__ cells,
                                                   const uint32_t* __restrict__ cand, size_t cand_frame_stride,
                                                   const int* __restrict__ cell_count, int n_cells,
                                                   uint32_t* __restrict__ scratch, size_t scratch_frame_stride,
                                                   int pool, int lds_keys_cap,
                                                   uint32_t* __restrict__ sel, int sel_frame_stride,
                                                   int* __restrict__ sel_count, int n_levels, int* __restrict__ status,
                                                   uint8_t* __restrict__ node_scratch, size_t node_stride, int level_first)
{
    extern __shared__ __align__(16) uint8_t smem[];
    __shared__ int s_sort_stack[3 * kIntrosortStack];
    const LevelDesc L = levels[level_first + blockIdx.x];
    const int* cc = cell_count + (size_t)blockIdx.y * n_cells + L.cell_begin;
    int total = 0;
    for (int ci = threadIdx.x; ci < L.cell_count; ci += 64) total += cc[ci];
    for (int o = 32; o > 0; o >>= 1) total += __shfl_xor(total, o);
    total = __builtin_amdgcn_readfirstlane(total);
    if (total <= lds_keys_cap)
        octree_body<true, true>(levels, cells, cand, cand_frame_stride, cell_count, n_cells, scratch, scratch_frame_stride, pool, lds_keys_cap,
                                sel, sel_frame_stride, sel_count, n_levels, status, node_scratch, node_stride, level_first, smem, s_sort_stack);
    else
        octree_body<false, true>(levels, cells, cand, cand_frame_stride, cell_count, n_cells, scratch, scratch_frame_stride, pool, lds_keys_cap,
                                 sel, sel_frame_stride, sel_count, n_levels, status, node_scratch, node_stride, level_first, smem, s_sort_stack);
}

__global__ __launch_bounds__(64) void k_debug_wave_sort(SortNode* __restrict__ data, int n)
{
    extern __shared__ __align__(16) uint8_t smem[];
    __shared__ int s_stack[3 * kIntrosortStack];
    SortNode* const v = (SortNode*)smem;
    SortNode* const out = v + n;
    short* const rank_tmp = (short*)(out + n);
    for (int i = threadIdx.x; i < n; i += 64) v[i] = data[i];
    __syncthreads();
    wave_sort_nodes(v, out, n, s_stack, rank_tmp);
    for (int i = threadIdx.x; i < n; i += 64) data[i] = out[i];
}

__global__ __launch_bounds__(64) void k_index(const LevelDesc* __restrict__ levels, int n_levels,
                                              const uint32_t* __restrict__ sel, int sel_frame_stride,
                                              const int* __restrict__ sel_count, int lap0, int lap1, int cap,
                                              int* __restrict__ kp_dst, int kp_frame_stride,
                                              int* __restrict__ n_out, int* __restrict__ mono_out, int* __restrict__ status)
{
    const int frame = blockIdx.x, lane = threadIdx.x;
    const int* sc = sel_count + (size_t)frame * n_levels;
    int total = 0;
    for (int l = 0; l < n_levels; l++) total += sc[l];
    int* dst = kp_dst + (size_t)frame * kp_frame_stride;
    int mono = 0, stereo = total - 1;
    const unsigned long long lt = (1ull << lane) - 1ull;
    for (int l = 0; l < n_levels; l++) {
        const LevelDesc L = levels[l];
        const uint32_t* s = sel + (size_t)frame * sel_frame_stride + L.sel_off;
        const int n = sc[l];
        for (int k0 = 0; k0 < n; k0 += 64) {
            const int k = k0 + lane;
            bool valid = k < n, lap = false;
            if (valid) {
                float x = (float)(key_x(s[k]) + 16);
                if (l != 0) x = x * L.scale;
                lap = (x >= (float)lap0) && (x <= (float)lap1);
            }
            const unsigned long long ml = __ballot(valid && lap), mm = __ballot(valid && !lap);
            if (valid) dst[L.sel_off + k] = lap ? stereo - __popcll(ml & lt) : mono + __popcll(mm & lt);
            stereo -= __popcll(ml);
            mono += __popcll(mm);
        }
    }
    if (lane == 0) {
        n_out[frame] = total;
        mono_out[frame] = mono;
        if (total > cap) atomicExch(status + frame, ORBX_ERR_CAPACITY);
    }
}

__device__ __forceinline__ int reflect101(int p, int len)
{
    if (len == 1) return 0;
    while (p < 0 || p >= len) p = (p < 0) ? -p : 2 * len - 2 - p;
    return p;
}

constexpr int kBlurTW = 64, kBlurTH = 58;

__global__ __launch_bounds__(256) void k_blur(SrcImage lvl0, const uint8_t* __restrict__ pyr, uint8_t* __restrict__ raw_out, uint8_t* __restrict__ blur,
                                              size_t frame_stride, const LevelDesc* __restrict__ levels, const TileDesc* __restrict__ tiles, int n_tiles,
                                              int t0, int t1, int t2, int t3)
{
    constexpr int SP = kBlurTW + 32, SR = kBlurTH + 6;
    __shared__ __align__(16) uint8_t s_src[SR * SP];
    __shared__ __align__(16) uint32_t s_hp[(SR / 2) * kBlurTW];
    const int tile_idx = xcd_remap(blockIdx.x, gridDim.x, blockIdx.y);
    if (tile_idx >= n_tiles) return;
    const TileDesc T = tiles[tile_idx];
    const LevelDesc L = levels[T.level];
    const bool ext = T.level == 0 && lvl0.base != nullptr;
    const uint8_t* img = ext ? lvl0.base + (size_t)blockIdx.y * lvl0.frame_stride : pyr + (size_t)blockIdx.y * frame_stride + L.off;
    const int istride = ext ? lvl0.stride : L.stride;
    uint8_t* dst = blur + (size_t)blockIdx.y * frame_stride + L.off;
    const int tid = threadIdx.x;
    const int x0 = T.x0, y0 = T.y0;
    for (int i = tid; i < SR * (SP / 16); i += 256) {
        const int r = i / (SP / 16), q = i - r * (SP / 16);
        const int sy = reflect101(y0 + r - 3, L.h), cx = x0 - 16 + 16 * q;
        uint4 v = make_uint4(0u, 0u, 0u, 0u);
        const uint8_t* rowp = img + (size_t)sy * istride;
        if (cx >= 0 && cx < L.w) v = *(const uint4*)(rowp + cx);
        if (cx < 0 || cx + 16 > L.w) {
            uint32_t w[4] = {v.x, v.y, v.z, v.w};
#pragma unroll
            for (int k = 1; k <= 3; k++) {
                const int bl = -k - cx, br = L.w - 1 + k - cx;
                if (bl >= 0 && bl < 16) { const uint32_t px = rowp[reflect101(-k, L.w)]; w[bl >> 2] = (w[bl >> 2] & ~(0xFFu << (8 * (bl & 3)))) | (px << (8 * (bl & 3))); }
                if (br >= 0 && br < 16) { const uint32_t px = rowp[reflect101(L.w - 1 + k, L.w)]; w[br >> 2] = (w[br >> 2] & ~(0xFFu << (8 * (br & 3)))) | (px << (8 * (br & 3))); }
            }
            v = make_uint4(w[0], w[1], w[2], w[3]);
        }
        *(uint4*)(s_src + r * SP + 16 * q) = v;
    }
    __syncthreads();
    if (ext && raw_out != nullptr) {
        uint8_t* raw = raw_out + (size_t)blockIdx.y * frame_stride + L.off;
        for (int i = tid; i < kBlurTH * (kBlurTW / 4); i += 256) {
            const int r = i >> 4, q = i & 15;
            if (y0 + r < L.h && x0 + 4 * q < L.w) *(uint32_t*)(raw + (size_t)(y0 + r) * L.stride + x0 + 4 * q) = *(const uint32_t*)(s_src + (r + 3) * SP + 16 + 4 * q);
        }
    }
    const uint32_t tapA = (uint32_t)t0 | ((uint32_t)t1 << 8) | ((uint32_t)t2 << 16) | ((uint32_t)t3 << 24);
    const uint32_t tapB = (uint32_t)t2 | ((uint32_t)t1 << 8) | ((uint32_t)t0 << 16);
    for (int i = tid; i < (SR / 2) * (kBlurTW / 4); i += 256) {
        const int p = i >> 4, q = i & 15;
        uint32_t o[2][4];
#pragma unroll
        for (int rr = 0; rr < 2; rr++) {
            const uint32_t* w = (const uint32_t*)(s_src + (2 * p + rr) * SP + 12) + q;
            const uint32_t w0 = w[0], w1 = w[1], w2 = w[2];
            o[rr][0] = __builtin_amdgcn_udot4(__builtin_amdgcn_alignbyte(w1, w0, 1), tapA, __builtin_amdgcn_udot4(__builtin_amdgcn_alignbyte(w2, w1, 1), tapB, 0u, false), false);
            o[rr][1] = __builtin_amdgcn_udot4(__builtin_amdgcn_alignbyte(w1, w0, 2), tapA, __builtin_amdgcn_udot4(__builtin_amdgcn_alignbyte(w2, w1, 2), tapB, 0u, false), false);
            o[rr][2] = __builtin_amdgcn_udot4(__builtin_amdgcn_alignbyte(w1, w0, 3), tapA, __builtin_amdgcn_udot4(__builtin_amdgcn_alignbyte(w2, w1, 3), tapB, 0u, false), false);
            o[rr][3] = __builtin_amdgcn_udot4(w1, tapA, __builtin_amdgcn_udot4(w2, tapB, 0u, false), false);
        }
        *(uint4*)(s_hp + p * kBlurTW + 4 * q) = make_uint4(o[0][0] | (o[1][0] << 16), o[0][1] | (o[1][1] << 16), o[0][2] | (o[1][2] << 16), o[0][3] | (o[1][3] << 16));
    }
    __syncthreads();
    const us2 cE0 = as_us2((uint32_t)t0 | ((uint32_t)t1 << 16)), cE1 = as_us2((uint32_t)t2 | ((uint32_t)t3 << 16)),
              cE2 = as_us2((uint32_t)t2 | ((uint32_t)t1 << 16)), cE3 = as_us2((uint32_t)t0);
    const us2 cO0 = as_us2((uint32_t)t0 << 16), cO1 = as_us2((uint32_t)t1 | ((uint32_t)t2 << 16)),
              cO2 = as_us2((uint32_t)t3 | ((uint32_t)t2 << 16)), cO3 = as_us2((uint32_t)t1 | ((uint32_t)t0 << 16));
    for (int i = tid; i < (kBlurTH / 2) * (kBlurTW / 4); i += 256) {
        const int m = i >> 4, q = i & 15;
        const int oy = y0 + 2 * m, ox = x0 + 4 * q;
        if (oy >= L.h || ox >= L.w) continue;
        const uint4 P0 = *(const uint4*)(s_hp + m * kBlurTW + 4 * q), P1 = *(const uint4*)(s_hp + (m + 1) * kBlurTW + 4 * q),
                    P2 = *(const uint4*)(s_hp + (m + 2) * kBlurTW + 4 * q), P3 = *(const uint4*)(s_hp + (m + 3) * kBlurTW + 4 * q);
        const uint32_t a0[4] = {P0.x, P0.y, P0.z, P0.w}, a1[4] = {P1.x, P1.y, P1.z, P1.w}, a2[4] = {P2.x, P2.y, P2.z, P2.w}, a3[4] = {P3.x, P3.y, P3.z, P3.w};
        uint32_t e[4], o[4];
#pragma unroll
        for (int k = 0; k < 4; k++) {
            e[k] = __builtin_amdgcn_udot2(as_us2(a3[k]), cE3, __builtin_amdgcn_udot2(as_us2(a2[k]), cE2, __builtin_amdgcn_udot2(as_us2(a1[k]), cE1,
                   __builtin_amdgcn_udot2(as_us2(a0[k]), cE0, 0x8000u, false), false), false), false);
            o[k] = __builtin_amdgcn_udot2(as_us2(a3[k]), cO3, __builtin_amdgcn_udot2(as_us2(a2[k]), cO2, __builtin_amdgcn_udot2(as_us2(a1[k]), cO1,
                   __builtin_amdgcn_udot2(as_us2(a0[k]), cO0, 0x8000u, false), false), false), false);
        }
        const uint32_t pe = __builtin_amdgcn_perm(__builtin_amdgcn_perm(e[3], e[2], 0x0C0C0602u), __builtin_amdgcn_perm(e[1], e[0], 0x0C0C0602u), 0x05040100u);
        const uint32_t po = __builtin_amdgcn_perm(__builtin_amdgcn_perm(o[3], o[2], 0x0C0C0602u), __builtin_amdgcn_perm(o[1], o[0], 0x0C0C0602u), 0x05040100u);
        *(uint32_t*)(dst + (size_t)oy * L.stride + ox) = pe;
        if (oy + 1 < L.h) *(uint32_t*)(dst + (size_t)(oy + 1) * L.stride + ox) = po;
    }
}

struct IcMask { uint32_t m[32][8]; };
constexpr IcMask make_ic_mask()
{
    IcMask t{};
    const int um[16] = {15, 15, 15, 15, 14, 14, 14, 13, 13, 12, 11, 10, 9, 8, 6, 3};
    for (int r = 0; r < 31; r++) {
        const int v = r - 15, av = v < 0 ? -v : v;
        for (int j = 0; j < 8; j++)
            for (int k = 0; k < 4; k++) {
                const int u = -15 + 4 * j + k, au = u < 0 ? -u : u;
                if (u <= 15 && au <= um[av]) t.m[r][j] |= 0xFFu << (8 * k);
            }
    }
    return t;
}
__device__ const IcMask d_ic_mask = make_ic_mask();

__global__ __launch_bounds__(256) void k_orient_desc(const uint8_t* __restrict__ pyr, const uint8_t* __restrict__ blur, size_t frame_stride,
                                                     const LevelDesc* __restrict__ levels, int n_levels,
                                                     const uint32_t* __restrict__ sel, int sel_frame_stride,
                                                     const int* __restrict__ sel_count,
                                                     const int* __restrict__ kp_dst, int kp_frame_stride,
                                                     OrbxKeyPoint* __restrict__ kps, uint8_t* __restrict__ desc, int cap,
                                                     OrbxKeyPoint* __restrict__ lvl_kps ,
                                                     int quads_per_frame, int batch)
{
    constexpr int kBR = 18, kBP = 64, kPR = 15;
    constexpr int kBBytes = (2 * kBR + 1) * kBP;
    __shared__ __align__(16) uint8_t s_patch[8][kBBytes];
    const int total_wg = gridDim.x, per_xcd = total_wg >> 3;
    const int v_id = (int)(blockIdx.x & 7) * per_xcd + (int)(blockIdx.x >> 3);
    const int frame = v_id / quads_per_frame, quad = v_id - frame * quads_per_frame;
    if (frame >= batch) return;
    const int lane = threadIdx.x & 63, wave = __builtin_amdgcn_readfirstlane(threadIdx.x >> 6);
    const int half = lane >> 5, hl = lane & 31;
    const int s_pair = quad * 8 + wave * 2, s_flat = s_pair + half;
    int level = 0;
    for (int l = 1; l < n_levels; l++) level = (s_pair >= levels[l].sel_off) ? l : level;
    const LevelDesc L = levels[level];
    const int k = s_flat - L.sel_off;
    const bool live = s_flat < sel_frame_stride && k < L.sel_cap && k < sel_count[(size_t)frame * n_levels + level];
    const int slot = L.sel_off + (live ? k : 0);
    const uint32_t e = live ? sel[(size_t)frame * sel_frame_stride + slot] : 0u;
    const int row = live ? kp_dst[(size_t)frame * kp_frame_stride + slot] : -1;
    uint32_t pw[8];
#pragma unroll
    for (int q = 0; q < 8; q++) pw[q] = ((const uint32_t*)d_pattern)[hl + 32 * q];
    const int px = (int)key_x(e) + 16, py = (int)key_y(e) + 16;
    uint8_t* sb = s_patch[wave * 2 + half];
    const int xb = (px - kBR) & ~15;
    uint32_t icw[9];
#pragma unroll
    for (int j = 0; j < 9; j++) icw[j] = 0u;
    if (live) {
        const uint8_t* bbase = blur + (size_t)frame * frame_stride + L.off + (size_t)(py - kBR) * L.stride + xb;
        for (int i = hl; i < (2 * kBR + 1) * 4; i += 32) {
            const int r = i >> 2, c = i & 3;
            *(uint4*)(sb + r * kBP + 16 * c) = *(const uint4*)(bbase + (size_t)r * L.stride + 16 * c);
        }
        if (hl < 2 * kPR + 1) {
            const uint8_t* rp = pyr + (size_t)frame * frame_stride + L.off + (size_t)(py - kPR + hl) * L.stride + ((px - kPR) & ~3);
            const Dwords4 q0 = *(const Dwords4*)rp, q1 = *(const Dwords4*)(rp + 16);
            icw[0] = q0.x; icw[1] = q0.y; icw[2] = q0.z; icw[3] = q0.w; icw[4] = q1.x; icw[5] = q1.y; icw[6] = q1.z; icw[7] = q1.w;
            icw[8] = *(const uint32_t*)(rp + 32);
        }
    }
    __builtin_amdgcn_fence(__ATOMIC_RELEASE, "wavefront");
    __builtin_amdgcn_wave_barrier();
    __builtin_amdgcn_fence(__ATOMIC_ACQUIRE, "wavefront");
    if (__ballot(live) == 0ull) return;

    int m10 = 0, m01 = 0;
    if (live && hl < 2 * kPR + 1) {
        const uint32_t sh = (uint32_t)((px - kPR) & 3);
        const uint4 ma = *(const uint4*)&d_ic_mask.m[hl][0], mb = *(const uint4*)&d_ic_mask.m[hl][4];
        const uint32_t mk[8] = {ma.x, ma.y, ma.z, ma.w, mb.x, mb.y, mb.z, mb.w};
        uint32_t a = 0u, b = 0u;
#pragma unroll
        for (int j = 0; j < 8; j++) {
            const uint32_t d = __builtin_amdgcn_alignbyte(icw[j + 1], icw[j], sh) & mk[j];
            a = __builtin_amdgcn_udot4(d, 0x01010101u, a, false);
            b = __builtin_amdgcn_udot4(d, 0x03020100u + 0x04040404u * (uint32_t)j, b, false);
        }
        m10 = (int)b - 15 * (int)a;
        m01 = (hl - kPR) * (int)a;
    }
    for (int o = 16; o > 0; o >>= 1) { m10 += __shfl_xor(m10, o); m01 += __shfl_xor(m01, o); }
    const float angle = fast_atan2_deg((float)m01, (float)m10);

    const float factorPI = (float)(3.141592653589793238462643383279502884 / 180.f);
    float a, b;
    sincos_f32(angle * factorPI, &a, &b);
    const uint8_t* bimg = sb + kBR * kBP + (px - xb);
    unsigned long long w[8];
#pragma unroll
    for (int q = 0; q < 8; q++) {
        const float x0 = (float)(signed char)(pw[q] & 0xFF), y0 = (float)(signed char)((pw[q] >> 8) & 0xFF);
        const float x1 = (float)(signed char)((pw[q] >> 16) & 0xFF), y1 = (float)(signed char)(pw[q] >> 24);
        int t0 = 0, t1 = 0;
        if (live) {
            t0 = bimg[cv_round_f(x0 * b + y0 * a) * kBP + cv_round_f(x0 * a - y0 * b)];
            t1 = bimg[cv_round_f(x1 * b + y1 * a) * kBP + cv_round_f(x1 * a - y1 * b)];
        }
        w[q] = __ballot(t0 < t1);
    }
    if (!live) return;
    if (hl == 0) {
        OrbxKeyPoint kp;
        kp.x = (float)px; kp.y = (float)py;
        kp.size = (float)L.patch_size; kp.angle = angle; kp.response = (float)key_resp(e);
        kp.octave = level; kp.class_id = -1;
        if (lvl_kps) lvl_kps[(size_t)frame * sel_frame_stride + slot] = kp;
        if (level != 0) { kp.x = kp.x * L.scale; kp.y = kp.y * L.scale; }
        if (row >= 0 && row < cap) kps[(size_t)frame * cap + row] = kp;
    }
    if (hl < 8 && row >= 0 && row < cap) {
        unsigned long long mine = w[0];
#pragma unroll
        for (int q = 1; q < 8; q++) mine = (hl == q) ? w[q] : mine;
        ((uint32_t*)(desc + ((size_t)frame * cap + row) * 32))[hl] = (uint32_t)(mine >> (32 * half));
    }
}

struct StereoTables { float scale[16], inv_scale[16]; };

__global__ __launch_bounds__(256) void k_stereo_match(const uint8_t* __restrict__ pyrL, const uint8_t* __restrict__ pyrR, size_t frame_stride,
                                                     const LevelDesc* __restrict__ levels, StereoTables T,
                                                     const OrbxKeyPoint* __restrict__ kpsL, const uint8_t* __restrict__ descL, const int32_t* __restrict__ nL,
                                                     const OrbxKeyPoint* __restrict__ kpsR, const uint8_t* __restrict__ descR, const int32_t* __restrict__ nR,
                                                     int cap, float mb, float mbf, int n_levels,
                                                     float* __restrict__ u_right, float* __restrict__ depth, int32_t* __restrict__ sad_out)
{
    __shared__ uint8_t s_l[4][11 * 12], s_r[4][11 * 24];
    __shared__ int s_part[4][11 * 11];
    const int frame = blockIdx.y, lane = threadIdx.x & 63, wave = threadIdx.x >> 6;
    const int iL = blockIdx.x * 4 + wave;
    const int n_l = min(nL[frame], cap), n_r = min(nR[frame], cap);
    const bool live = iL < n_l;
    const size_t fo = (size_t)frame * cap;
    float uL = 0, vL = 0;
    int levelL = 0;
    unsigned key = 0xFFFFFFFFu;
    if (live) {
        const OrbxKeyPoint kl = kpsL[fo + iL];
        uL = kl.x; vL = kl.y; levelL = kl.octave;
        const int v_row = (int)vL;
        const float minZ = mb, minD = 0, maxD = mbf / minZ;
        const float minU = uL - maxD, maxU = uL - minD;
        const unsigned long long* dl = (const unsigned long long*)(descL + (fo + iL) * 32);
        const unsigned long long d0 = dl[0], d1 = dl[1], d2 = dl[2], d3 = dl[3];
        for (int iR = lane; iR < n_r; iR += 64) {
            const OrbxKeyPoint kr = kpsR[fo + iR];
            const float r = 2.0f * T.scale[kr.octave & 15];
            const int maxr = (int)ceilf(kr.y + r), minr = (int)floorf(kr.y - r);
            if (v_row < minr || v_row > maxr) continue;
            if (kr.octave < levelL - 1 || kr.octave > levelL + 1) continue;
            if (!(kr.x >= minU && kr.x <= maxU)) continue;
            const unsigned long long* dr = (const unsigned long long*)(descR + (fo + iR) * 32);
            const int dist = __popcll(d0 ^ dr[0]) + __popcll(d1 ^ dr[1]) + __popcll(d2 ^ dr[2]) + __popcll(d3 ^ dr[3]);
            if (dist < 100) key = min(key, ((unsigned)dist << 20) | (unsigned)iR);
        }
    }
    for (int o = 32; o > 0; o >>= 1) key = min(key, (unsigned)__shfl_xor((int)key, o));
    const int thOrbDist = (100 + 50) / 2;
    bool ok = live && key != 0xFFFFFFFFu && (int)(key >> 20) < thOrbDist;
    if (levelL < 0 || levelL >= n_levels) ok = false;
    float scaleduR0 = 0;
    int y0 = 0, xl0 = 0, xr_start = 0;
    size_t loff = 0;
    int lstride = 0;
    if (ok) {
        const float uR0 = kpsR[fo + (key & 0xFFFFFu)].x;
        const float scaleFactor = T.inv_scale[levelL & 15];
        const float scaleduL = roundf(uL * scaleFactor), scaledvL = roundf(vL * scaleFactor);
        scaleduR0 = roundf(uR0 * scaleFactor);
        const LevelDesc L = levels[levelL];
        loff = (size_t)L.off; lstride = L.stride;
        const int w = 5, Ls = 5;
        const float iniu = scaleduR0 + Ls - w, endu = scaleduR0 + Ls + w + 1;
        if (iniu < 0 || endu >= (float)L.w) ok = false;
        y0 = (int)(scaledvL - w); xl0 = (int)(scaleduL - w); xr_start = (int)(scaleduR0 - Ls - w);
        if (y0 < 0 || y0 + 11 > L.h || xl0 < 0 || xl0 + 11 > L.w || xr_start < 0 || xr_start + 21 > L.w) ok = false;
    }
    if (ok) {
        const uint8_t* il = pyrL + (size_t)frame * frame_stride + loff;
        const uint8_t* ir = pyrR + (size_t)frame * frame_stride + loff;
        for (int i = lane; i < 121; i += 64) { const int r = i / 11, c = i - r * 11; s_l[wave][r * 12 + c] = il[(size_t)(y0 + r) * lstride + xl0 + c]; }
        for (int i = lane; i < 231; i += 64) { const int r = i / 21, c = i - r * 21; s_r[wave][r * 24 + c] = ir[(size_t)(y0 + r) * lstride + xr_start + c]; }
    }
    __syncthreads();
    if (ok) {
        for (int i = lane; i < 121; i += 64) {
            const int sft = i / 11, r = i - sft * 11;
            int acc = 0;
#pragma unroll
            for (int c = 0; c < 11; c++) acc += abs((int)s_l[wave][r * 12 + c] - (int)s_r[wave][r * 24 + sft + c]);
            s_part[wave][sft * 11 + r] = acc;
        }
    }
    __syncthreads();
    if (ok && lane == 0) {
        const int Ls = 5;
        float vDists[11];
        int bestDist = 0x7FFFFFFF, bestincR = 0;
        for (int sft = 0; sft < 11; sft++) {
            int sad = 0;
            for (int r = 0; r < 11; r++) sad += s_part[wave][sft * 11 + r];
            const float dist = (float)sad;
            if (dist < (float)bestDist) { bestDist = (int)dist; bestincR = sft - Ls; }
            vDists[sft] = dist;
        }
        float ur_out = -1.0f, depth_out = -1.0f;
        int sad_best = -1;
        if (!(bestincR == -Ls || bestincR == Ls)) {
            const float dist1 = vDists[Ls + bestincR - 1], dist2 = vDists[Ls + bestincR], dist3 = vDists[Ls + bestincR + 1];
            const float deltaR = (dist1 - dist3) / (2.0f * (dist1 + dist3 - 2.0f * dist2));
            if (!(deltaR < -1 || deltaR > 1)) {
                float bestuR = T.scale[levelL & 15] * ((float)scaleduR0 + (float)bestincR + deltaR);
                float disparity = (uL - bestuR);
                const float minD = 0, maxD = mbf / mb;
                if (disparity >= minD && disparity < maxD) {
                    if (disparity <= 0) { disparity = 0.01; bestuR = uL - 0.01; }
                    depth_out = mbf / disparity;
                    ur_out = bestuR;
                    sad_best = bestDist;
                }
            }
        }
        u_right[fo + iL] = ur_out; depth[fo + iL] = depth_out; sad_out[fo + iL] = sad_best;
    } else if (live && lane == 0) {
        u_right[fo + iL] = -1.0f; depth[fo + iL] = -1.0f; sad_out[fo + iL] = -1;
    }
}

__global__ __launch_bounds__(256) void k_stereo_median(const int32_t* __restrict__ nL, int cap, int n_pow2_max,
                                                      float* __restrict__ u_right, float* __restrict__ depth, const int32_t* __restrict__ sad)
{
    extern __shared__ int s_sad[];
    __shared__ int s_cnt;
    const int frame = blockIdx.x, tid = threadIdx.x;
    const int n = min(nL[frame], cap);
    int n_pow2 = 2;
    while (n_pow2 < n) n_pow2 <<= 1;
    n_pow2 = min(n_pow2, n_pow2_max);
    const size_t fo = (size_t)frame * cap;
    if (tid == 0) s_cnt = 0;
    __syncthreads();
    int local = 0;
    for (int i = tid; i < n_pow2; i += 256) {
        const int v = (i < n) ? sad[fo + i] : -1;
        s_sad[i] = v >= 0 ? v : 0x7FFFFFFF;
        local += v >= 0;
    }
    if (local) atomicAdd(&s_cnt, local);
    __syncthreads();
    {
        const int lane = tid & 63, wave = tid >> 6;
        const int chunk = n_pow2 >> 2, pairs = n_pow2 >> 3;
        bool need_block = false;
        for (int k = 2; k <= n_pow2; k <<= 1)
            for (int j = k >> 1; j > 0; j >>= 1) {
                const bool cross = j >= chunk || n_pow2 < 8;
                if (cross || need_block) __syncthreads();
                else { __builtin_amdgcn_fence(__ATOMIC_RELEASE, "wavefront"); __builtin_amdgcn_wave_barrier(); __builtin_amdgcn_fence(__ATOMIC_ACQUIRE, "wavefront"); }
                need_block = cross;
                const int t0 = n_pow2 >= 8 ? wave * pairs + lane : tid, t1 = n_pow2 >= 8 ? (wave + 1) * pairs : (n_pow2 >> 1), ts = n_pow2 >= 8 ? 64 : 256;
                for (int t = t0; t < t1; t += ts) {
                    const int lo = 2 * t - (t & (j - 1)), hi = lo + j;
                    const bool up = (lo & k) == 0;
                    const int a = s_sad[lo], b = s_sad[hi];
                    if ((a > b) == up) { s_sad[lo] = b; s_sad[hi] = a; }
                }
            }
        __syncthreads();
    }
    const int m = s_cnt;
    if (m == 0) return;
    const float median = (float)s_sad[m / 2];
    const float thDist = 1.5f * 1.4f * median;
    for (int i = tid; i < n; i += 256) {
        const int v = sad[fo + i];
        if (v >= 0 && !((float)v < thDist)) { u_right[fo + i] = -1; depth[fo + i] = -1; }
    }
}

}
```

Baseline: 266,700 frames/s.

## Streamline resize and blur kernels with packed row tables and 32-bit addressing

Resize now reads a packed per-row table (source rows plus pre-shifted beta weights) with one 16-byte load per row. It uses 24-bit multiplies for offsets instead of 64-bit size_t math, and hoists the boundary check out of the row loop. The blur tile load is restructured so each thread loads one 16-byte chunk plus halo words, with reflect padding done only on edge tiles flagged at setup time. The raw level-0 copy is folded into that load, and the loop-based h/v passes become fixed two-item-per-thread helpers. The change adds 2 GiB size guards to keep the 32-bit offsets valid, at the cost of limiting the image and pyramid size.

```diff
diff --git a/orb_slam3-1_amd/csrc/orbx_device.h b/orb_slam3-1_amd/csrc/orbx_device.h
--- a/orb_slam3-1_amd/csrc/orbx_device.h
+++ b/orb_slam3-1_amd/csrc/orbx_device.h
@@ -31,7 +31,12 @@
 };
 
 struct TileDesc {
-    int16_t level, x0, y0, pad;
+    int16_t level, x0, y0;
+    int16_t edge;
+};
+
+struct __attribute__((aligned(16))) ResizeRow {
+    uint32_t sy, b0, b1, pad;
 };
 
 __host__ __device__ inline int xcd_grid(int n_items) { return 8 * ((n_items + 7) / 8); }
diff --git a/orb_slam3-1_amd/csrc/orbx_extractor.hip b/orb_slam3-1_amd/csrc/orbx_extractor.hip
--- a/orb_slam3-1_amd/csrc/orbx_extractor.hip
+++ b/orb_slam3-1_amd/csrc/orbx_extractor.hip
@@ -108,11 +108,11 @@
     DevBuf<CellDesc> d_cells;
     DevBuf<TileDesc> d_tiles;
     DevBuf<StripDesc> d_strips;
-    std::vector<DevBuf<int> > d_qsx0, d_yofs;
+    std::vector<DevBuf<int> > d_qsx0;
     std::vector<DevBuf<uint4> > d_qsel, d_qalpha;
-    std::vector<DevBuf<short> > d_ibeta;
-    std::vector<DevBuf<int> > d_xofs;
-    std::vector<DevBuf<short> > d_ialpha;
+    std::vector<DevBuf<ResizeRow> > d_rows;
+    std::vector<DevBuf<int> > d_xofs, d_yofs;
+    std::vector<DevBuf<short> > d_ialpha, d_ibeta;
     std::vector<uint8_t> resize_generic;
 
     int batch_cap = 0, last_batch = 0;
@@ -197,7 +197,7 @@
     size_t off = 0;
     int cand_off = 0, sel_off = 0, max_tw = 0, max_th = 0, max_nfeat = 0;
     std::vector<int> node_need(nlevels, 0);
-    d_qsx0.resize(nlevels); d_yofs.resize(nlevels); d_qsel.resize(nlevels); d_qalpha.resize(nlevels); d_ibeta.resize(nlevels);
+    d_qsx0.resize(nlevels); d_yofs.resize(nlevels); d_qsel.resize(nlevels); d_qalpha.resize(nlevels); d_ibeta.resize(nlevels); d_rows.resize(nlevels);
     d_xofs.resize(nlevels); d_ialpha.resize(nlevels); resize_generic.assign(nlevels, 0);
     for (int l = 0; l < nlevels; l++) {
         LevelDesc& L = levels[l];
@@ -272,7 +272,8 @@
         }
         for (int y0 = 0; y0 < L.h; y0 += kBlurTH)
             for (int x0 = 0; x0 < L.w; x0 += kBlurTW) {
-                TileDesc t; t.level = (int16_t)l; t.x0 = (int16_t)x0; t.y0 = (int16_t)y0; t.pad = 0;
+                TileDesc t; t.level = (int16_t)l; t.x0 = (int16_t)x0; t.y0 = (int16_t)y0;
+                t.edge = (int16_t)((x0 == 0 ? 1 : 0) | (L.w <= x0 + kBlurTW + 2 ? 2 : 0));
                 tiles.push_back(t);
             }
         if (l > 0) {
@@ -319,13 +320,22 @@
                 qsel[q] = make_uint4(se[0], se[1], se[2], se[3]);
                 qal[q] = make_uint4(al[0], al[1], al[2], al[3]);
             }
+            std::vector<ResizeRow> rows((size_t)round_up(L.h, kResizeRows));
+            for (size_t dy = 0; dy < rows.size(); dy++) {
+                const int y = std::min((int)dy, L.h - 1);
+                const int sy0 = std::min(std::max(yofs[y], 0), P.h - 1), sy1 = std::min(std::max(yofs[y] + 1, 0), P.h - 1);
+                if (ib[2 * y] < 0 || ib[2 * y] > 2048 || ib[2 * y + 1] < 0 || ib[2 * y + 1] > 2048)
+                    return fail(ORBX_ERR_INTERNAL, "resize table: row coefficients %d %d", ib[2 * y], ib[2 * y + 1]);
+                rows[dy].sy = (uint32_t)sy0 | ((uint32_t)sy1 << 16);
+                rows[dy].b0 = (uint32_t)ib[2 * y] << 12; rows[dy].b1 = (uint32_t)ib[2 * y + 1] << 12; rows[dy].pad = 0;
+            }
             int r;
-            if (resize_generic[l] && ((r = d_xofs[l].upload(xofs)) || (r = d_ialpha[l].upload(ia)))) return r;
-            if ((r = d_qsx0[l].upload(qsx0)) || (r = d_yofs[l].upload(yofs)) || (r = d_qsel[l].upload(qsel)) || (r = d_qalpha[l].upload(qal)) ||
-                (r = d_ibeta[l].upload(ib))) return r;
+            if (resize_generic[l] && ((r = d_xofs[l].upload(xofs)) || (r = d_ialpha[l].upload(ia)) || (r = d_yofs[l].upload(yofs)) || (r = d_ibeta[l].upload(ib)))) return r;
+            if ((r = d_qsx0[l].upload(qsx0)) || (r = d_qsel[l].upload(qsel)) || (r = d_qalpha[l].upload(qal)) || (r = d_rows[l].upload(rows))) return r;
         }
     }
     pyr_frame_bytes = off;
+    if (off >= ((size_t)1 << 31)) return fail(ORBX_ERR_ARG, "the pyramid of a %dx%d image exceeds 2 GiB per frame", w, h);
     cand_frame_entries = std::max(cand_off, 1);
     sel_frame_entries = sel_off;
     {
@@ -495,7 +505,7 @@
                                    d_xofs[l].p, d_ialpha[l].p, d_yofs[l].p, d_ibeta[l].p);
             else
             hipLaunchKernelGGL(k_resize, g, dim3(256), 0, rs, src, pyr, pyr_frame_bytes, D,
-                               d_qsx0[l].p, d_qsel[l].p, d_qalpha[l].p, d_yofs[l].p, d_ibeta[l].p);
+                               d_qsx0[l].p, d_qsel[l].p, d_qalpha[l].p, d_rows[l].p);
             ORBX_LAUNCHED("k_resize");
         }
         if (chain_beside) ORBX_HIP(hipEventRecord(ev_resize, rs));
@@ -535,7 +545,7 @@
         if (l_tail < nlevels) {
             ResizeTables T;
             std::memset(&T, 0, sizeof(T));
-            for (int l = l_tail; l < nlevels; l++) { T.q_sx0[l] = d_qsx0[l].p; T.q_sel[l] = d_qsel[l].p; T.q_alpha[l] = d_qalpha[l].p; T.yofs[l] = d_yofs[l].p; T.ibeta[l] = d_ibeta[l].p; }
+            for (int l = l_tail; l < nlevels; l++) { T.q_sx0[l] = d_qsx0[l].p; T.q_sel[l] = d_qsel[l].p; T.q_alpha[l] = d_qalpha[l].p; T.rows[l] = d_rows[l].p; }
             const bool beside = blur_s && oct_stream && n_cells > 0 && tail_strip > 0;
             hipStream_t ts = beside ? oct_stream : s;
             if (beside && !chain_beside) { ORBX_HIP(hipEventRecord(ev_fork, s)); ORBX_HIP(hipStreamWaitEvent(ts, ev_fork, 0)); }
@@ -734,6 +744,7 @@
     for (auto& b : e->d_qsel) b.release();
     for (auto& b : e->d_qalpha) b.release();
     for (auto& b : e->d_ibeta) b.release();
+    for (auto& b : e->d_rows) b.release();
     for (auto& b : e->d_xofs) b.release();
     for (auto& b : e->d_ialpha) b.release();
     e->d_pyr.release(); e->d_blur.release(); e->d_cand.release(); e->d_scratch.release(); e->d_sel.release(); e->d_oct_nodes.release();
@@ -786,6 +797,8 @@
 {
     if (!e || !d_imgs || !d_kps || !d_desc || !d_n || !d_mono || !d_status) return fail(ORBX_ERR_ARG, "NULL argument");
     if (batch < 1 || width < 1 || height < 1 || row_stride < width || cap < 1) return fail(ORBX_ERR_ARG, "bad batch/geometry");
+    if (row_stride >= (1 << 24) || (uint64_t)row_stride * (uint64_t)height >= (1ull << 31))
+        return fail(ORBX_ERR_ARG, "a frame of %d rows of %d bytes exceeds 2 GiB (or a row 16 MiB)", height, row_stride);
     ORBX_HIP(hipSetDevice(e->device));
     int r;
     if ((r = e->setup_geometry(width, height)) || (r = e->ensure_batch(batch))) return r;
diff --git a/orb_slam3-1_amd/csrc/orbx_kernels.hip b/orb_slam3-1_amd/csrc/orbx_kernels.hip
--- a/orb_slam3-1_amd/csrc/orbx_kernels.hip
+++ b/orb_slam3-1_amd/csrc/orbx_kernels.hip
@@ -21,52 +21,54 @@
     int32_t stride, w, h;
 };
 
+__device__ __forceinline__ uint32_t mul_hi_u24(uint32_t a, uint32_t b) { return (uint32_t)(((uint64_t)(a & 0xFFFFFFu) * (uint64_t)(b & 0xFFFFFFu)) >> 32); }
+
 struct __attribute__((aligned(4))) Dwords3 { uint32_t x, y, z; };
 struct __attribute__((aligned(4))) Dwords4 { uint32_t x, y, z, w; };
 constexpr int kResizeRows = 64, kResizeTW = 64;
 
-__device__ __forceinline__ void resize_tile(const SrcImage& src, uint8_t* __restrict__ pyr, size_t frame_stride, const LevelDesc& dst,
+__device__ __forceinline__ void resize_tile(const uint8_t* __restrict__ S, int s_stride, uint8_t* __restrict__ D, const LevelDesc& dst,
                                             const int* __restrict__ q_sx0, const uint4* __restrict__ q_sel, const uint4* __restrict__ q_alpha,
-                                            const int* __restrict__ yofs, const short* __restrict__ ibeta, int tile, int frame, int lane, int wave)
+                                            const ResizeRow* __restrict__ rows, int tile, int lane, int wave)
 {
     const int tiles_x = (dst.w + kResizeTW - 1) / kResizeTW;
     const int ty = tile / tiles_x, tx = tile - ty * tiles_x;
     const int q = tx * (kResizeTW / 4) + (lane & 15), rsel = lane >> 4;
     if (4 * q >= dst.w) return;
+    constexpr int NR = kResizeRows / 16;
+    const int dy0 = ty * kResizeRows + wave * (kResizeRows / 4) + rsel;
+    ResizeRow rw[NR];
+#pragma unroll
+    for (int r = 0; r < NR; r++) rw[r] = *(const ResizeRow*)((const uint8_t*)rows + (((uint32_t)dy0 << 4) + 64u * r));
     const int sx0 = q_sx0[q];
     const uint4 sel = q_sel[q], al = q_alpha[q];
     const uint32_t sels[4] = {sel.x, sel.y, sel.z, sel.w}, als[4] = {al.x, al.y, al.z, al.w};
-    const int a = sx0 & ~3;
+    const uint32_t a = (uint32_t)(sx0 & ~3);
     const uint32_t sh = (uint32_t)(sx0 & 3);
-    const int last = src.stride - 4;
-    const int o0 = a, o1 = min(a + 4, last), o2 = min(a + 8, last);
-    const uint8_t* S = src.base + (size_t)frame * src.frame_stride;
-    uint8_t* D = pyr + (size_t)frame * frame_stride + dst.off + 4 * q;
-    constexpr int NR = kResizeRows / 16;
-    const int dy0 = ty * kResizeRows + wave * (kResizeRows / 4) + rsel;
-    uint32_t u[NR][3], v[NR][3], bb[NR];
-#pragma unroll
-    for (int r = 0; r < NR; r++) {
-        const int dy = min(dy0 + 4 * r, dst.h - 1);
-        const int sy = yofs[dy];
-        const int sy0 = min(max(sy, 0), src.h - 1), sy1 = min(max(sy + 1, 0), src.h - 1);
-        bb[r] = ((const uint32_t*)ibeta)[dy];
-        const uint8_t* r0p = S + (size_t)sy0 * src.stride;
-        const uint8_t* r1p = S + (size_t)sy1 * src.stride;
-        if (a + 8 <= last) {
-            const Dwords3 tu = *(const Dwords3*)(r0p + a), tv = *(const Dwords3*)(r1p + a);
+    const uint32_t last = (uint32_t)(s_stride - 4);
+    uint32_t u[NR][3], v[NR][3], r0[NR], r1[NR];
+#pragma unroll
+    for (int r = 0; r < NR; r++) { r0[r] = __umul24(rw[r].sy & 0xFFFFu, (uint32_t)s_stride) + a; r1[r] = __umul24(rw[r].sy >> 16, (uint32_t)s_stride) + a; }
+    if (a + 8 <= last) {
+#pragma unroll
+        for (int r = 0; r < NR; r++) {
+            const Dwords3 tu = *(const Dwords3*)(S + r0[r]), tv = *(const Dwords3*)(S + r1[r]);
             u[r][0] = tu.x; u[r][1] = tu.y; u[r][2] = tu.z;
             v[r][0] = tv.x; v[r][1] = tv.y; v[r][2] = tv.z;
-        } else {
-            u[r][0] = *(const uint32_t*)(r0p + o0); u[r][1] = *(const uint32_t*)(r0p + o1); u[r][2] = *(const uint32_t*)(r0p + o2);
-            v[r][0] = *(const uint32_t*)(r1p + o0); v[r][1] = *(const uint32_t*)(r1p + o1); v[r][2] = *(const uint32_t*)(r1p + o2);
-        }
-    }
+        }
+    } else {
+        const uint32_t d1 = min(a + 4, last) - a, d2 = min(a + 8, last) - a;
+#pragma unroll
+        for (int r = 0; r < NR; r++) {
+            u[r][0] = *(const uint32_t*)(S + r0[r]); u[r][1] = *(const uint32_t*)(S + (r0[r] + d1)); u[r][2] = *(const uint32_t*)(S + (r0[r] + d2));
+            v[r][0] = *(const uint32_t*)(S + r1[r]); v[r][1] = *(const uint32_t*)(S + (r1[r] + d1)); v[r][2] = *(const uint32_t*)(S + (r1[r] + d2));
+        }
+    }
+    const uint32_t off0 = __umul24((uint32_t)dy0, (uint32_t)dst.stride) + 4u * (uint32_t)q;
 #pragma unroll
     for (int r = 0; r < NR; r++) {
-        const int dy = dy0 + 4 * r;
-        if (dy >= dst.h) continue;
-        const uint32_t b0 = bb[r] & 0xFFFFu, b1 = bb[r] >> 16;
+        if (dy0 + 4 * r >= dst.h) continue;
+        const uint32_t b0 = rw[r].b0, b1 = rw[r].b1;
         const uint32_t ulo = __builtin_amdgcn_alignbyte(u[r][1], u[r][0], sh), uhi = __builtin_amdgcn_alignbyte(u[r][2], u[r][1], sh);
         const uint32_t vlo = __builtin_amdgcn_alignbyte(v[r][1], v[r][0], sh), vhi = __builtin_amdgcn_alignbyte(v[r][2], v[r][1], sh);
         uint32_t out[4];
@@ -75,22 +77,21 @@
             const us2 ak = as_us2(als[k]);
             const uint32_t h0 = __builtin_amdgcn_udot2(as_us2(__builtin_amdgcn_perm(uhi, ulo, sels[k])), ak, 0u, false);
             const uint32_t h1 = __builtin_amdgcn_udot2(as_us2(__builtin_amdgcn_perm(vhi, vlo, sels[k])), ak, 0u, false);
-            const uint32_t val = ((__umul24(b0, h0 >> 4) >> 16) + (__umul24(b1, h1 >> 4) >> 16) + 2u) >> 2;
-            out[k] = min(val, 255u);
-        }
-        *(uint32_t*)(D + (size_t)dy * dst.stride) = out[0] | (out[1] << 8) | (out[2] << 16) | (out[3] << 24);
+            out[k] = min((mul_hi_u24(b0, h0 & ~15u) + mul_hi_u24(b1, h1 & ~15u) + 2u) >> 2, 255u);
+        }
+        *(uint32_t*)(D + (off0 + (uint32_t)(4 * r) * (uint32_t)dst.stride)) = out[0] | (out[1] << 8) | (out[2] << 16) | (out[3] << 24);
     }
 }
 
 __global__ __launch_bounds__(256) void k_resize(SrcImage src, uint8_t* __restrict__ pyr, size_t frame_stride, LevelDesc dst,
                                                 const int* __restrict__ q_sx0, const uint4* __restrict__ q_sel, const uint4* __restrict__ q_alpha,
-                                                const int* __restrict__ yofs, const short* __restrict__ ibeta)
+                                                const ResizeRow* __restrict__ rows)
 {
     const int tiles_x = (dst.w + kResizeTW - 1) / kResizeTW, tiles_y = (dst.h + kResizeRows - 1) / kResizeRows;
     const int tile = xcd_remap(blockIdx.x, gridDim.x, blockIdx.y);
     if (tile >= tiles_x * tiles_y) return;
-    resize_tile(src, pyr, frame_stride, dst, q_sx0, q_sel, q_alpha, yofs, ibeta, tile, blockIdx.y, threadIdx.x & 63,
-                __builtin_amdgcn_readfirstlane(threadIdx.x >> 6));
+    resize_tile(src.base + (size_t)blockIdx.y * src.frame_stride, src.stride, pyr + (size_t)blockIdx.y * frame_stride + dst.off, dst,
+                q_sx0, q_sel, q_alpha, rows, tile, threadIdx.x & 63, __builtin_amdgcn_readfirstlane(threadIdx.x >> 6));
 }
 
 __global__ __launch_bounds__(256) void k_resize_generic(SrcImage src, uint8_t* __restrict__ pyr, size_t frame_stride, LevelDesc dst,
@@ -114,7 +115,7 @@
 
 struct ResizeTables {
     const int* q_sx0[kMaxLevels]; const uint4* q_sel[kMaxLevels]; const uint4* q_alpha[kMaxLevels];
-    const int* yofs[kMaxLevels]; const short* ibeta[kMaxLevels];
+    const ResizeRow* rows[kMaxLevels];
 };
 __global__ __launch_bounds__(1024) void k_resize_tail(uint8_t* __restrict__ pyr, size_t frame_stride, const LevelDesc* __restrict__ levels,
                                                       ResizeTables T, int l_first, int n_levels)
@@ -124,11 +125,10 @@
     const int lane = threadIdx.x & 63;
     for (int l = l_first; l < n_levels; l++) {
         const LevelDesc D = levels[l], P = levels[l - 1];
-        SrcImage src;
-        src.base = pyr + P.off; src.frame_stride = frame_stride; src.stride = P.stride; src.w = P.w; src.h = P.h;
+        uint8_t* fp = pyr + (size_t)frame * frame_stride;
         const int tiles = ((D.w + kResizeTW - 1) / kResizeTW) * ((D.h + kResizeRows - 1) / kResizeRows);
         for (int t = sub; t < tiles; t += 4)
-            resize_tile(src, pyr, frame_stride, D, T.q_sx0[l], T.q_sel[l], T.q_alpha[l], T.yofs[l], T.ibeta[l], t, frame, lane, wave);
+            resize_tile(fp + P.off, P.stride, fp + D.off, D, T.q_sx0[l], T.q_sel[l], T.q_alpha[l], T.rows[l], t, lane, wave);
         __syncthreads();
     }
 }
@@ -612,12 +612,49 @@
 }
 
 constexpr int kBlurTW = 64, kBlurTH = 58;
+constexpr int kBlurSP = 96;
+
+__device__ __forceinline__ void blur_h_item(const uint8_t* __restrict__ src , uint32_t* __restrict__ hp, uint32_t tapA, uint32_t tapB)
+{
+    uint32_t o[2][4];
+#pragma unroll
+    for (int rr = 0; rr < 2; rr++) {
+        const uint32_t* w = (const uint32_t*)(src + rr * kBlurSP);
+        const uint32_t w0 = w[0], w1 = w[1], w2 = w[2];
+        o[rr][0] = __builtin_amdgcn_udot4(__builtin_amdgcn_alignbyte(w1, w0, 1), tapA, __builtin_amdgcn_udot4(__builtin_amdgcn_alignbyte(w2, w1, 1), tapB, 0u, false), false);
+        o[rr][1] = __builtin_amdgcn_udot4(__builtin_amdgcn_alignbyte(w1, w0, 2), tapA, __builtin_amdgcn_udot4(__builtin_amdgcn_alignbyte(w2, w1, 2), tapB, 0u, false), false);
+        o[rr][2] = __builtin_amdgcn_udot4(__builtin_amdgcn_alignbyte(w1, w0, 3), tapA, __builtin_amdgcn_udot4(__builtin_amdgcn_alignbyte(w2, w1, 3), tapB, 0u, false), false);
+        o[rr][3] = __builtin_amdgcn_udot4(w1, tapA, __builtin_amdgcn_udot4(w2, tapB, 0u, false), false);
+    }
+    *(uint4*)hp = make_uint4(__builtin_amdgcn_perm(o[1][0], o[0][0], 0x05040100u), __builtin_amdgcn_perm(o[1][1], o[0][1], 0x05040100u),
+                             __builtin_amdgcn_perm(o[1][2], o[0][2], 0x05040100u), __builtin_amdgcn_perm(o[1][3], o[0][3], 0x05040100u));
+}
+
+struct BlurTaps { us2 e0, e1, e2, e3, o0, o1, o2, o3; };
+
+__device__ __forceinline__ void blur_v_item(const uint32_t* __restrict__ hp, const BlurTaps& c, uint8_t* __restrict__ dst, uint32_t off, uint32_t stride, bool odd_row)
+{
+    const uint4 P0 = *(const uint4*)hp, P1 = *(const uint4*)(hp + kBlurTW), P2 = *(const uint4*)(hp + 2 * kBlurTW), P3 = *(const uint4*)(hp + 3 * kBlurTW);
+    const uint32_t a0[4] = {P0.x, P0.y, P0.z, P0.w}, a1[4] = {P1.x, P1.y, P1.z, P1.w}, a2[4] = {P2.x, P2.y, P2.z, P2.w}, a3[4] = {P3.x, P3.y, P3.z, P3.w};
+    uint32_t e[4], o[4];
+#pragma unroll
+    for (int k = 0; k < 4; k++) {
+        e[k] = __builtin_amdgcn_udot2(as_us2(a3[k]), c.e3, __builtin_amdgcn_udot2(as_us2(a2[k]), c.e2, __builtin_amdgcn_udot2(as_us2(a1[k]), c.e1,
+               __builtin_amdgcn_udot2(as_us2(a0[k]), c.e0, 0x8000u, false), false), false), false);
+        o[k] = __builtin_amdgcn_udot2(as_us2(a3[k]), c.o3, __builtin_amdgcn_udot2(as_us2(a2[k]), c.o2, __builtin_amdgcn_udot2(as_us2(a1[k]), c.o1,
+               __builtin_amdgcn_udot2(as_us2(a0[k]), c.o0, 0x8000u, false), false), false), false);
+    }
+    const uint32_t pe = __builtin_amdgcn_perm(__builtin_amdgcn_perm(e[3], e[2], 0x0C0C0602u), __builtin_amdgcn_perm(e[1], e[0], 0x0C0C0602u), 0x05040100u);
+    const uint32_t po = __builtin_amdgcn_perm(__builtin_amdgcn_perm(o[3], o[2], 0x0C0C0602u), __builtin_amdgcn_perm(o[1], o[0], 0x0C0C0602u), 0x05040100u);
+    *(uint32_t*)(dst + off) = pe;
+    if (odd_row) *(uint32_t*)(dst + (off + stride)) = po;
+}
 
 __global__ __launch_bounds__(256) void k_blur(SrcImage lvl0, const uint8_t* __restrict__ pyr, uint8_t* __restrict__ raw_out, uint8_t* __restrict__ blur,
                                               size_t frame_stride, const LevelDesc* __restrict__ levels, const TileDesc* __restrict__ tiles, int n_tiles,
                                               int t0, int t1, int t2, int t3)
 {
-    constexpr int SP = kBlurTW + 32, SR = kBlurTH + 6;
+    constexpr int SP = kBlurSP, SR = kBlurTH + 6;
     __shared__ __align__(16) uint8_t s_src[SR * SP];
     __shared__ __align__(16) uint32_t s_hp[(SR / 2) * kBlurTW];
     const int tile_idx = xcd_remap(blockIdx.x, gridDim.x, blockIdx.y);
@@ -626,76 +663,66 @@
     const LevelDesc L = levels[T.level];
     const bool ext = T.level == 0 && lvl0.base != nullptr;
     const uint8_t* img = ext ? lvl0.base + (size_t)blockIdx.y * lvl0.frame_stride : pyr + (size_t)blockIdx.y * frame_stride + L.off;
-    const int istride = ext ? lvl0.stride : L.stride;
+    const uint32_t istride = (uint32_t)(ext ? lvl0.stride : L.stride), ostride = (uint32_t)L.stride;
     uint8_t* dst = blur + (size_t)blockIdx.y * frame_stride + L.off;
     const int tid = threadIdx.x;
-    const int x0 = T.x0, y0 = T.y0;
-    for (int i = tid; i < SR * (SP / 16); i += 256) {
-        const int r = i / (SP / 16), q = i - r * (SP / 16);
-        const int sy = reflect101(y0 + r - 3, L.h), cx = x0 - 16 + 16 * q;
+    const int x0 = T.x0, y0 = T.y0, w = L.w, h = L.h;
+    const int rows_in = min(h - y0, kBlurTH);
+    {
+        const int r = tid >> 2, c = tid & 3;
+        const int cx = x0 + 16 * c, y = y0 + r - 3;
         uint4 v = make_uint4(0u, 0u, 0u, 0u);
-        const uint8_t* rowp = img + (size_t)sy * istride;
-        if (cx >= 0 && cx < L.w) v = *(const uint4*)(rowp + cx);
-        if (cx < 0 || cx + 16 > L.w) {
-            uint32_t w[4] = {v.x, v.y, v.z, v.w};
-#pragma unroll
-            for (int k = 1; k <= 3; k++) {
-                const int bl = -k - cx, br = L.w - 1 + k - cx;
-                if (bl >= 0 && bl < 16) { const uint32_t px = rowp[reflect101(-k, L.w)]; w[bl >> 2] = (w[bl >> 2] & ~(0xFFu << (8 * (bl & 3)))) | (px << (8 * (bl & 3))); }
-                if (br >= 0 && br < 16) { const uint32_t px = rowp[reflect101(L.w - 1 + k, L.w)]; w[br >> 2] = (w[br >> 2] & ~(0xFFu << (8 * (br & 3)))) | (px << (8 * (br & 3))); }
-            }
-            v = make_uint4(w[0], w[1], w[2], w[3]);
-        }
-        *(uint4*)(s_src + r * SP + 16 * q) = v;
+        uint32_t left = 0u, right = 0u;
+        if (r < rows_in + 6) {
+            const uint32_t ro = __umul24((uint32_t)reflect101(y, h), istride);
+            if (cx < w) v = *(const uint4*)(img + (ro + (uint32_t)cx));
+            if (c == 0 && x0 > 0) left = *(const uint32_t*)(img + (ro + (uint32_t)(x0 - 4)));
+            if (c == 3 && x0 + kBlurTW < w) right = *(const uint32_t*)(img + (ro + (uint32_t)(x0 + kBlurTW)));
+            *(uint4*)(s_src + r * SP + 16 + 16 * c) = v;
+            if (c == 0) *(uint32_t*)(s_src + r * SP + 12) = left;
+            if (c == 3) *(uint32_t*)(s_src + r * SP + 16 + kBlurTW) = right;
+            if (ext && raw_out != nullptr && r >= 3 && r < rows_in + 3 && cx < w) {
+                uint8_t* rp = raw_out + (size_t)blockIdx.y * frame_stride + L.off + (__umul24((uint32_t)y, ostride) + (uint32_t)cx);
+                if (cx + 12 < w) *(uint4*)rp = v;
+                else {
+                    *(uint32_t*)rp = v.x;
+                    if (cx + 4 < w) *(uint32_t*)(rp + 4) = v.y;
+                    if (cx + 8 < w) *(uint32_t*)(rp + 8) = v.z;
+                }
+            }
+        }
     }
     __syncthreads();
-    if (ext && raw_out != nullptr) {
-        uint8_t* raw = raw_out + (size_t)blockIdx.y * frame_stride + L.off;
-        for (int i = tid; i < kBlurTH * (kBlurTW / 4); i += 256) {
-            const int r = i >> 4, q = i & 15;
-            if (y0 + r < L.h && x0 + 4 * q < L.w) *(uint32_t*)(raw + (size_t)(y0 + r) * L.stride + x0 + 4 * q) = *(const uint32_t*)(s_src + (r + 3) * SP + 16 + 4 * q);
-        }
+    if (T.edge) {
+        const int r = tid & 63, j = __builtin_amdgcn_readfirstlane(tid >> 6);
+        if (j < 3) {
+            uint8_t* row = s_src + r * SP + 16 - x0;
+            if (T.edge & 1) row[-1 - j] = row[reflect101(-1 - j, w)];
+            if ((T.edge & 2) && w + j < x0 + kBlurTW + 4) row[w + j] = row[reflect101(w + j, w)];
+        }
+        __syncthreads();
     }
     const uint32_t tapA = (uint32_t)t0 | ((uint32_t)t1 << 8) | ((uint32_t)t2 << 16) | ((uint32_t)t3 << 24);
     const uint32_t tapB = (uint32_t)t2 | ((uint32_t)t1 << 8) | ((uint32_t)t0 << 16);
-    for (int i = tid; i < (SR / 2) * (kBlurTW / 4); i += 256) {
-        const int p = i >> 4, q = i & 15;
-        uint32_t o[2][4];
-#pragma unroll
-        for (int rr = 0; rr < 2; rr++) {
-            const uint32_t* w = (const uint32_t*)(s_src + (2 * p + rr) * SP + 12) + q;
-            const uint32_t w0 = w[0], w1 = w[1], w2 = w[2];
-            o[rr][0] = __builtin_amdgcn_udot4(__builtin_amdgcn_alignbyte(w1, w0, 1), tapA, __builtin_amdgcn_udot4(__builtin_amdgcn_alignbyte(w2, w1, 1), tapB, 0u, false), false);
-            o[rr][1] = __builtin_amdgcn_udot4(__builtin_amdgcn_alignbyte(w1, w0, 2), tapA, __builtin_amdgcn_udot4(__builtin_amdgcn_alignbyte(w2, w1, 2), tapB, 0u, false), false);
-            o[rr][2] = __builtin_amdgcn_udot4(__builtin_amdgcn_alignbyte(w1, w0, 3), tapA, __builtin_amdgcn_udot4(__builtin_amdgcn_alignbyte(w2, w1, 3), tapB, 0u, false), false);
-            o[rr][3] = __builtin_amdgcn_udot4(w1, tapA, __builtin_amdgcn_udot4(w2, tapB, 0u, false), false);
-        }
-        *(uint4*)(s_hp + p * kBlurTW + 4 * q) = make_uint4(o[0][0] | (o[1][0] << 16), o[0][1] | (o[1][1] << 16), o[0][2] | (o[1][2] << 16), o[0][3] | (o[1][3] << 16));
+    const int q = tid & 15, pm = tid >> 4;
+    const bool q_in = x0 + 4 * q < w;
+    {
+        const uint8_t* sp = s_src + 2 * pm * SP + 12 + 4 * q;
+        uint32_t* hp = s_hp + pm * kBlurTW + 4 * q;
+        if (q_in && 2 * pm < rows_in + 6) blur_h_item(sp, hp, tapA, tapB);
+        if (q_in && 2 * pm + 32 < rows_in + 6) blur_h_item(sp + 32 * SP, hp + 16 * kBlurTW, tapA, tapB);
     }
     __syncthreads();
-    const us2 cE0 = as_us2((uint32_t)t0 | ((uint32_t)t1 << 16)), cE1 = as_us2((uint32_t)t2 | ((uint32_t)t3 << 16)),
-              cE2 = as_us2((uint32_t)t2 | ((uint32_t)t1 << 16)), cE3 = as_us2((uint32_t)t0);
-    const us2 cO0 = as_us2((uint32_t)t0 << 16), cO1 = as_us2((uint32_t)t1 | ((uint32_t)t2 << 16)),
-              cO2 = as_us2((uint32_t)t3 | ((uint32_t)t2 << 16)), cO3 = as_us2((uint32_t)t1 | ((uint32_t)t0 << 16));
-    for (int i = tid; i < (kBlurTH / 2) * (kBlurTW / 4); i += 256) {
-        const int m = i >> 4, q = i & 15;
-        const int oy = y0 + 2 * m, ox = x0 + 4 * q;
-        if (oy >= L.h || ox >= L.w) continue;
-        const uint4 P0 = *(const uint4*)(s_hp + m * kBlurTW + 4 * q), P1 = *(const uint4*)(s_hp + (m + 1) * kBlurTW + 4 * q),
-                    P2 = *(const uint4*)(s_hp + (m + 2) * kBlurTW + 4 * q), P3 = *(const uint4*)(s_hp + (m + 3) * kBlurTW + 4 * q);
-        const uint32_t a0[4] = {P0.x, P0.y, P0.z, P0.w}, a1[4] = {P1.x, P1.y, P1.z, P1.w}, a2[4] = {P2.x, P2.y, P2.z, P2.w}, a3[4] = {P3.x, P3.y, P3.z, P3.w};
-        uint32_t e[4], o[4];
-#pragma unroll
-        for (int k = 0; k < 4; k++) {
-            e[k] = __builtin_amdgcn_udot2(as_us2(a3[k]), cE3, __builtin_amdgcn_udot2(as_us2(a2[k]), cE2, __builtin_amdgcn_udot2(as_us2(a1[k]), cE1,
-                   __builtin_amdgcn_udot2(as_us2(a0[k]), cE0, 0x8000u, false), false), false), false);
-            o[k] = __builtin_amdgcn_udot2(as_us2(a3[k]), cO3, __builtin_amdgcn_udot2(as_us2(a2[k]), cO2, __builtin_amdgcn_udot2(as_us2(a1[k]), cO1,
-                   __builtin_amdgcn_udot2(as_us2(a0[k]), cO0, 0x8000u, false), false), false), false);
-        }
-        const uint32_t pe = __builtin_amdgcn_perm(__builtin_amdgcn_perm(e[3], e[2], 0x0C0C0602u), __builtin_amdgcn_perm(e[1], e[0], 0x0C0C0602u), 0x05040100u);
-        const uint32_t po = __builtin_amdgcn_perm(__builtin_amdgcn_perm(o[3], o[2], 0x0C0C0602u), __builtin_amdgcn_perm(o[1], o[0], 0x0C0C0602u), 0x05040100u);
-        *(uint32_t*)(dst + (size_t)oy * L.stride + ox) = pe;
-        if (oy + 1 < L.h) *(uint32_t*)(dst + (size_t)(oy + 1) * L.stride + ox) = po;
+    {
+        BlurTaps c;
+        c.e0 = as_us2((uint32_t)t0 | ((uint32_t)t1 << 16)); c.e1 = as_us2((uint32_t)t2 | ((uint32_t)t3 << 16));
+        c.e2 = as_us2((uint32_t)t2 | ((uint32_t)t1 << 16)); c.e3 = as_us2((uint32_t)t0);
+        c.o0 = as_us2((uint32_t)t0 << 16); c.o1 = as_us2((uint32_t)t1 | ((uint32_t)t2 << 16));
+        c.o2 = as_us2((uint32_t)t3 | ((uint32_t)t2 << 16)); c.o3 = as_us2((uint32_t)t1 | ((uint32_t)t0 << 16));
+        const uint32_t* hp = s_hp + pm * kBlurTW + 4 * q;
+        const uint32_t off = __umul24((uint32_t)(y0 + 2 * pm), ostride) + (uint32_t)(x0 + 4 * q);
+        if (q_in && 2 * pm < rows_in) blur_v_item(hp, c, dst, off, ostride, 2 * pm + 1 < rows_in);
+        if (q_in && 2 * pm + 32 < rows_in) blur_v_item(hp + 16 * kBlurTW, c, dst, off + 32u * ostride, ostride, 2 * pm + 33 < rows_in);
     }
 }
 
```

Result: faster. 271,700 frames/s, median of 6 (+1.9%).
